# p-mc-grath/DMMFODS

Measured on AMD Instinct MI355X. Metric: training images/sec at 1280x1920 RGB+LiDAR, higher is better.
Workload: dtype f16; 1 GPU; C2 d121 early-fusion 6ch b4 1280x1920; key=c2, per_gpu_batch=4, global_batch=4, height=1280, width=1920, storage_dtype=fp16, accumulate=fp32, parallelism=dp1, weights=random-init (reference init, seed 123)

## Files before the change

### dmmfods_amd/_lib.py

```python
import ctypes as C
import os

_HERE = os.path.dirname(os.path.abspath(__file__))
LIB_PATH = os.environ.get("DMM_LIB_PATH") or os.path.join(_HERE, "libdmmfods_hip.so")

DMM_F32, DMM_F16, DMM_BF16 = 0, 1, 2
LOSS_BCE, LOSS_FOCAL = 0, 1
T_CONV, T_CONVT, T_BN_WEIGHT, T_BN_BIAS, T_BN_MEAN, T_BN_VAR, T_BN_TRACKED = range(7)
ERR_INVALID, ERR_SHAPE, ERR_HIP, ERR_STATE, ERR_NO_DEVICE = -1, -2, -3, -4, -5


class ModelDesc(C.Structure):
    _fields_ = [
        ("growth_rate", C.c_int32), ("num_blocks", C.c_int32), ("block_config", C.c_int32 * 8),
        ("num_init_features", C.c_int32), ("bn_size", C.c_int32), ("num_classes", C.c_int32),
        ("concat_before_block_num", C.c_int32), ("stream_1_in_channels", C.c_int32),
        ("stream_2_in_channels", C.c_int32), ("batch", C.c_int32), ("height", C.c_int32), ("width", C.c_int32),
        ("dtype", C.c_int32), ("loss_scale", C.c_float), ("bn_momentum", C.c_float), ("bn_eps", C.c_float),
        ("iou_threshold", C.c_float), ("use_mfma", C.c_int32),
    ]


class ConvDesc(C.Structure):
    _fields_ = [(n, C.c_int32) for n in (
        "dtype", "use_mfma", "B", "H", "W", "Cin", "Cout", "R", "S", "stride", "pad", "transposed", "mode", "bn_relu")]


class GuardState(C.Structure):
    _fields_ = [("scale", C.c_float), ("grad_scale", C.c_float), ("sumsq", C.c_double), ("grad_norm", C.c_float),
                ("found_inf", C.c_int32), ("applied_steps", C.c_int64), ("skipped_steps", C.c_int64),
                ("growth_tracker", C.c_int32), ("step_size", C.c_float), ("bc2_sqrt", C.c_float), ("clip_coef", C.c_float),
                ("reserved", C.c_int32 * 2)]


assert C.sizeof(GuardState) == 64

ADAM_MAX_CLASSES = 16


class AdamSegment(C.Structure):
    _fields_ = [("begin", C.c_int64), ("count", C.c_int64), ("cls", C.c_int32)]


class AdamClass(C.Structure):
    _fields_ = [("lr", C.c_float), ("beta1", C.c_float), ("beta2", C.c_float), ("eps", C.c_float), ("weight_decay", C.c_float),
                ("decoupled", C.c_int32), ("t0", C.c_int64)]


assert C.sizeof(AdamSegment) == 24 and C.sizeof(AdamClass) == 32


class DmmError(RuntimeError):
    pass


_lib = None


def lib():
    global _lib
    if _lib is not None:
        return _lib
    if not os.path.exists(LIB_PATH):
        raise ImportError(
            f"{LIB_PATH} is missing: build it with `python -c 'import __graft_entry__ as g; g.build()'` "
            "(or `make -C dmmfods_amd/csrc`).  dmmfods_amd has no CPU fallback.")
    import torch
    tl = os.path.join(os.path.dirname(torch.__file__), "lib", "libamdhip64.so")
    if os.path.exists(tl):
        C.CDLL(tl, mode=C.RTLD_GLOBAL)
    L = C.CDLL(LIB_PATH)
    vp, i32, i64, f32, sz = C.c_void_p, C.c_int32, C.c_int64, C.c_float, C.c_size_t
    L.dmm_last_error.restype = C.c_char_p
    L.dmm_version.restype = C.c_int
    L.dmm_last_impl.restype = C.c_int
    L.dmm_impl_name.restype = C.c_char_p
    L.dmm_impl_name.argtypes = [C.c_int]
    L.dmm_impl_mask.restype = C.c_uint
    L.dmm_impl_mask.argtypes = [C.c_int]
    L.dmm_set_option.restype = C.c_int
    L.dmm_set_option.argtypes = [C.c_char_p, C.c_int]
    L.dmm_plan_create.argtypes = [C.POINTER(ModelDesc), C.POINTER(vp)]
    L.dmm_plan_destroy.argtypes = [vp]
    L.dmm_plan_destroy.restype = C.c_int
    L.dmm_plan_num_tensors.argtypes = [vp]
    L.dmm_plan_tensor_info.argtypes = [vp, C.c_int, C.POINTER(C.c_char_p), C.POINTER(i32), C.POINTER(i32),
                                       C.POINTER(i64 * 4), C.POINTER(i64)]
    L.dmm_plan_num_params.argtypes = [vp]
    L.dmm_plan_num_params.restype = i64
    L.dmm_plan_num_buffer_elems.argtypes = [vp]
    L.dmm_plan_num_buffer_elems.restype = i64
    L.dmm_plan_workspace_bytes.argtypes = [vp]
    L.dmm_plan_workspace_bytes.restype = sz
    L.dmm_plan_forward_flops.argtypes = [vp]
    L.dmm_plan_forward_flops.restype = C.c_double
    L.dmm_plan_bind.argtypes = [vp, vp, sz, vp, vp, vp]
    L.dmm_plan_forward.argtypes = [vp, vp, vp, vp, C.c_int, vp]
    L.dmm_plan_loss_backward.argtypes = [vp, vp, vp, vp, vp]
    L.dmm_plan_backward.argtypes = [vp, vp, vp]
    L.dmm_plan_loss_metrics.argtypes = [vp, vp, vp, vp, vp]
    L.dmm_plan_set_loss.argtypes = [vp, C.c_int, vp, vp, C.c_int]
    L.dmm_loss_forward.argtypes = [C.c_int, C.c_int, vp, vp, vp, vp, vp, vp, C.c_int, C.c_int, C.c_int, C.c_int, vp]
    L.dmm_plan_num_grad_buckets.argtypes = [vp]
    L.dmm_plan_num_graph_replays.argtypes = [vp, C.c_int]
    L.dmm_plan_num_graph_replays.restype = C.c_longlong
    L.dmm_plan_grad_bucket.argtypes = [vp, C.c_int, C.POINTER(i64), C.POINTER(i64)]
    L.dmm_plan_grad_bucket_wait.argtypes = [vp, C.c_int, vp]
    L.dmm_plan_profile_begin.argtypes = [vp, C.c_int]
    L.dmm_plan_profile_filter.restype = C.c_int
    L.dmm_plan_profile_filter.argtypes = [vp, C.c_char_p]
    L.dmm_plan_profile_num_ops.argtypes = [vp, C.c_int]
    L.dmm_plan_profile_op.argtypes = [vp, C.c_int, C.c_int, C.POINTER(C.c_char_p), C.POINTER(C.c_double), C.POINTER(C.c_double)]
    L.dmm_plan_profile_collect.argtypes = [vp, C.c_int, C.POINTER(C.c_double), C.c_int, C.POINTER(C.c_int)]
    L.dmm_adam_step.argtypes = [vp, vp, vp, vp, i64, f32, f32, f32, f32, f32, i64, f32, vp]
    L.dmm_grad_guard_scratch_bytes.argtypes = [i64]
    L.dmm_grad_guard_scratch_bytes.restype = sz
    L.dmm_guard_state_init.argtypes = [vp, f32, i64, i32, vp]
    L.dmm_adam_step_guarded.argtypes = [vp, vp, vp, vp, i64, f32, f32, f32, f32, f32, f32, f32, f32, i32, vp, vp, vp]
    L.dmm_adam_step_guarded_ranges.argtypes = [vp, vp, vp, vp, C.POINTER(i64), C.POINTER(i64), C.POINTER(i64), C.c_int,
                                               f32, f32, f32, f32, f32, f32, f32, f32, i32, vp, vp, vp]
    L.dmm_plan_set_encoder_frozen.argtypes = [vp, C.c_int]
    L.dmm_adam_table_bytes.argtypes = [C.c_int, i64]
    L.dmm_adam_table_bytes.restype = sz
    L.dmm_adam_table_init.argtypes = [vp, C.POINTER(AdamSegment), C.c_int, i64, C.c_int, vp]
    L.dmm_adam_step_segmented.argtypes = [vp, vp, vp, vp, i64, vp, C.c_int, C.POINTER(AdamClass), C.c_int, i64, f32, vp]
    L.dmm_adam_step_guarded_segmented.argtypes = [vp, vp, vp, vp, i64, vp, C.c_int, C.POINTER(AdamClass), C.c_int, f32, f32, f32, i32,
                                                  vp, vp, vp]
    L.dmm_grad_sumsq.argtypes = [vp, i64, i64, C.c_int, vp, vp]
    L.dmm_plan_set_dynamic_loss_scale.argtypes = [vp, vp]
    L.dmm_plan_set_grad_accumulate.argtypes = [vp, C.c_int]
    L.dmm_conv_scratch_bytes.argtypes = [C.POINTER(ConvDesc)]
    L.dmm_conv_scratch_bytes.restype = sz
    L.dmm_conv_forward.argtypes = [C.POINTER(ConvDesc), vp, vp, vp, vp, vp, vp, vp, vp]
    L.dmm_conv_wgrad.argtypes = [C.POINTER(ConvDesc), vp, vp, vp, vp, vp, vp, vp]
    L.dmm_conv_dgrad.argtypes = [C.POINTER(ConvDesc), vp, vp, vp, vp, vp, vp, vp, vp, vp]
    L.dmm_conv_wgrad_ex.argtypes = [C.POINTER(ConvDesc), vp, vp, vp, vp, vp, vp, vp, C.c_int, vp, vp, vp]
    L.dmm_conv_dgrad_ex.argtypes = [C.POINTER(ConvDesc), vp, vp, vp, vp, vp, vp, vp, vp, vp, C.c_int, vp, vp, vp]
    L.dmm_conv1x1_backward_fused.argtypes = [C.POINTER(ConvDesc), vp, vp, vp, vp, vp, vp, vp, vp, vp, C.c_int, vp, vp, vp, vp]
    L.dmm_conv5_wgrad_stats.argtypes = [C.POINTER(ConvDesc), vp, vp, vp, vp, vp, vp, vp, vp, vp]
    L.dmm_plan_wgrad_batch_counts.argtypes = [vp, C.POINTER(C.c_longlong * 4)]
    L.dmm_conv_wgrad_grouped.argtypes = [C.POINTER(ConvDesc), C.c_int, vp, vp, vp, vp, vp, vp, vp, vp, vp, C.c_int, C.POINTER(C.c_int), vp]
    L.dmm_bw1_reduce_grouped.argtypes = [C.c_int, vp, vp, C.POINTER(C.c_int), C.POINTER(C.c_int), C.POINTER(C.c_int), C.c_int,
                                         C.POINTER(C.c_int), vp]
    _lib = L
    return L


EXPORTS = [
    "dmm_last_error", "dmm_version", "dmm_set_option", "dmm_plan_create", "dmm_plan_destroy", "dmm_plan_num_tensors",
    "dmm_plan_tensor_info", "dmm_plan_num_params", "dmm_plan_num_buffer_elems", "dmm_plan_workspace_bytes",
    "dmm_plan_forward_flops", "dmm_plan_bind", "dmm_plan_forward", "dmm_plan_loss_backward", "dmm_plan_backward",
    "dmm_plan_loss_metrics", "dmm_plan_num_graph_replays", "dmm_plan_set_loss", "dmm_loss_forward", "dmm_plan_num_grad_buckets", "dmm_plan_grad_bucket",
    "dmm_plan_grad_bucket_wait", "dmm_plan_profile_begin", "dmm_plan_profile_filter", "dmm_plan_profile_num_ops", "dmm_plan_profile_op",
    "dmm_plan_profile_collect", "dmm_adam_step", "dmm_conv_scratch_bytes", "dmm_conv_forward", "dmm_conv_wgrad",
    "dmm_conv_dgrad", "dmm_conv_wgrad_ex", "dmm_conv_dgrad_ex", "dmm_conv1x1_backward_fused", "dmm_conv5_wgrad_stats", "dmm_last_impl", "dmm_impl_name", "dmm_impl_mask",
    "dmm_grad_guard_scratch_bytes", "dmm_guard_state_init", "dmm_adam_step_guarded", "dmm_grad_sumsq", "dmm_plan_set_dynamic_loss_scale",
    "dmm_plan_set_grad_accumulate", "dmm_plan_set_encoder_frozen", "dmm_adam_step_guarded_ranges",
    "dmm_adam_table_bytes", "dmm_adam_table_init", "dmm_adam_step_segmented", "dmm_adam_step_guarded_segmented",
    "dmm_plan_wgrad_batch_counts", "dmm_conv_wgrad_grouped", "dmm_bw1_reduce_grouped",
]


def check(rc):
    if rc == 0:
        return
    msg = lib().dmm_last_error().decode(errors="replace")
    if rc == ERR_SHAPE:
        raise ValueError(msg)
    if rc == ERR_INVALID and "fusion" in msg:
        raise AttributeError(msg)
    if rc == ERR_INVALID:
        raise ValueError(msg)
    raise DmmError(f"dmm status {rc}: {msg}")


def last_impl():
    L = lib()
    return L.dmm_impl_name(L.dmm_last_impl()).decode()


def impls_since_reset(reset=True):
    L = lib()
    m = L.dmm_impl_mask(1 if reset else 0)
    return {L.dmm_impl_name(i).decode() for i in range(32) if (m >> i) & 1}


def stream_ptr():
    import torch
    return C.c_void_p(torch.cuda.current_stream().cuda_stream)
```

### dmmfods_amd/csrc/bw1.hip

```cpp
#include <algorithm>
#include <cstdio>
#include <cstring>
#include <cstdlib>
#include <type_traits>

#include "common.h"
#include "dispatch.h"
#include "gather.h"
#include "isa.h"
#include "pointwise.h"

namespace dmm {

#ifndef B1_DBG
#define B1_DBG 0
#endif
#ifndef B1_LATE_PREFETCH
#define B1_LATE_PREFETCH 0
#endif
#ifndef B1_RAW_BAR
#define B1_RAW_BAR 0
#endif
#ifndef B1_NT
#define B1_NT 0
#endif
#ifndef B1_GOLD_EARLY
#define B1_GOLD_EARLY 0
#endif
constexpr int B1_TM = 64;
constexpr int B1_NB = 128;
constexpr int B1_CT = 128;
constexpr int B1_IMG = B1_TM * 256;
constexpr int B1_W = 4 * B1_CT * 64;
constexpr int B1_STAGE = B1_TM * B1_CT * 4;
static_assert(B1_STAGE == 2 * B1_IMG, "staging aliases the operand images exactly");
constexpr int B1_LDS = 2 * B1_IMG + B1_W + 2 * B1_CT * 8 + 6 * B1_CT * 4;

__device__ __forceinline__ int b1_swz(int row, int slot) { return ((((slot >> 2) ^ (row & 3)) << 2) | ((slot & 3) ^ ((row >> 2) & 3))); }

template <typename T, int PQ, bool ACC_, bool PART>
__global__ __launch_bounds__(NTHREADS, 2) void bw1_kernel(const Bw1Args g) {
  constexpr bool ACC = ACC_ && !(B1_DBG & 32);
  constexpr bool UNC = std::is_same<T, f16>::value;
  static_assert(sizeof(T) == 2, "16-bit storage");
  typedef typename TT<T>::vec V;
  constexpr int SLOT = 8;
  constexpr int NL = B1_TM * 16 / NTHREADS;
  const ConvArgs& a = g.c;
  const Seg& sg = a.seg[0];

  extern __shared__ __attribute__((aligned(16))) unsigned char smem[];
  unsigned char* Ai = smem;
  unsigned char* Gi = smem + B1_IMG;
  unsigned char* Wi = smem + 2 * B1_IMG;
  double* red = (double*)(smem + 2 * B1_IMG + B1_W);
  float* kc = (float*)(smem + 2 * B1_IMG + B1_W + 2 * B1_CT * 8);

  const int tid = threadIdx.x, lane = tid & 63, wave = tid >> 6;
  const int r = lane & 31, h = lane >> 5;
  const int xcd = blockIdx.x & 7, q = blockIdx.x >> 3;
  const int ct = g.xcd_group ? q % g.nct : (int)(blockIdx.x % g.nct);
  const int split = g.xcd_group ? (q / g.nct) * 8 + xcd : (int)(blockIdx.x / g.nct);
  const int c0 = ct * B1_CT;
  const int t_beg = split * g.tiles_per_wg, t_end = min(g.ntiles, t_beg + g.tiles_per_wg);
  if (t_beg >= t_end) return;

  const int cs = tid & 15, p0 = tid >> 4;
  const int cx = c0 + cs * SLOT;
  const bool cvalid = cx < a.N;
  if (tid < B1_CT) {
    const int c = c0 + tid;
    const bool v = c < a.N;
    kc[tid] = v ? a.bscale[c] : 0.f; kc[B1_CT + tid] = v ? a.bshift[c] : 0.f;
    kc[2 * B1_CT + tid] = v ? a.bmean[c] : 0.f; kc[3 * B1_CT + tid] = v ? a.binvstd[c] : 0.f;
    kc[4 * B1_CT + tid] = PQ == 2 ? sg.q[tid] : 0.f; kc[5 * B1_CT + tid] = PQ == 2 ? sg.r[tid] : 0.f;
  }
  const unsigned char* xbase = (const unsigned char*)a.bx;
  const unsigned char* gbase = (const unsigned char*)sg.src;
  const unsigned char* ybase = (const unsigned char*)sg.src2;
  unsigned char* obase = (unsigned char*)a.out;
  const unsigned xcol = (unsigned)(cvalid ? cx : 0) * 2u, gcol = (unsigned)(cs * SLOT) * 2u;
  const unsigned xpitch = (unsigned)a.ldbx * 2u, gpitch = (unsigned)sg.ld * 2u, ypitch = (unsigned)sg.ld2 * 2u, opitch = (unsigned)a.ldo * 2u;
  const int lds0 = p0 * 256 + (b1_swz(p0, cs) << 4);

  {
    const T* wp = (const T*)a.wpack;
#pragma unroll
    for (int j = 0; j < B1_W / 16 / NTHREADS; ++j) {
      const int piece = tid + NTHREADS * j;
      const int chunk = piece >> 9, rowc = (piece >> 2) & 127, slot = piece & 3;
      const int c = c0 + rowc;
      V v;
#pragma unroll
      for (int e = 0; e < SLOT; ++e) v[e] = (T)0;
      if (c < a.Npad) v = *(const V*)(wp + ((size_t)chunk * a.Npad + c) * 32 + slot * SLOT);
      *(V*)(Wi + chunk * (B1_CT * 64) + rowc * 64 + ((slot ^ ((rowc >> 2) & 3)) << 4)) = v;
    }
  }
  if (tid < 2 * B1_CT) red[tid] = 0.0;
  __syncthreads();

  V rx[NL], rg[NL], ry[PQ == 2 ? NL : 1];
  unsigned okp = 0;
  auto issue = [&](int tile) {
    okp = 0;
#pragma unroll
    for (int i = 0; i < NL; ++i) {
      const int m = tile * B1_TM + p0 + 16 * i;
      if (m < a.M) okp |= 1u << i;
      const unsigned mm = (B1_DBG & 16) ? 0u : (unsigned)min(m, a.M - 1);
      if (B1_NT & 1) rx[i] = __builtin_nontemporal_load((const V*)(xbase + (size_t)(mm * xpitch + xcol)));
      else rx[i] = *(const V*)(xbase + (size_t)(mm * xpitch + xcol));
      rg[i] = *(const V*)(gbase + (size_t)(mm * gpitch + gcol));
      if constexpr (PQ == 2) ry[i] = *(const V*)(ybase + (size_t)(mm * ypitch + gcol));
    }
  };

  const int dpx = 32 * (wave & 1) + r;
  const int dgoff = dpx * 256;
  const int dcb = 64 * (wave >> 1);
  const int bsw = (r >> 2) & 3;
  const int tg = lane >> 4, ti = lane & 15, tq = ti >> 2, tp = ti & 3;
  const int arow = 8 * (tg >> 1) + tq;
  auto tr_off = [&](int px, int colbyte) { return px * 256 + ((b1_swz(px, colbyte >> 4) << 4) | (colbyte & 15)); };
  const int acolb = (32 * wave + 16 * (tg & 1) + 4 * tp) * 2;
  const int aoff1 = tr_off(arow, acolb);
  int goff1[4];
#pragma unroll
  for (int j = 0; j < 4; ++j) goff1[j] = tr_off(arow, (32 * j + 16 * (tg & 1) + 4 * tp) * 2);
  auto second = [](int off) { return (off ^ 16) + 4 * 256; };

  f32x16 accw[4];
#pragma unroll
  for (int j = 0; j < 4; ++j)
#pragma unroll
    for (int i = 0; i < 16; ++i) accw[j][i] = 0.f;

  issue(t_beg);
  for (int tile = t_beg; tile < t_end; ++tile) {
    V xraw[NL], gold[ACC ? NL : 1];
    const bool full = (tile + 1) * B1_TM <= a.M;
    const unsigned okt = okp;
    auto stage = [&](auto full_tag) {
      constexpr bool FULL = decltype(full_tag)::value;
      V z;
#pragma unroll
      for (int e = 0; e < SLOT; ++e) z[e] = (T)0;
      {
        SlotK<SLOT> kx;
        kx.k0 = load_fv<SLOT>(kc + cs * SLOT); kx.k1 = load_fv<SLOT>(kc + B1_CT + cs * SLOT); kx.k2 = 0.f; kx.k3 = 0.f;
#pragma unroll
        for (int i = 0; i < NL; ++i) {
          xraw[i] = rx[i];
          const bool v = FULL || ((okt >> i) & 1) != 0;
          const V av_ = bn_relu_slot(rx[i], kx);
          *(V*)(Ai + lds0 + 4096 * i) = v ? av_ : z;
        }
      }
      {
        SlotK<SLOT> kg;
        kg.k0 = 0.f; kg.k1 = 0.f; kg.k2 = 0.f; kg.k3 = 0.f;
        if (PQ == 2) { kg.k0 = load_fv<SLOT>(kc + 4 * B1_CT + cs * SLOT); kg.k1 = load_fv<SLOT>(kc + 5 * B1_CT + cs * SLOT); }
#pragma unroll
        for (int i = 0; i < NL; ++i) {
          const bool v = FULL || ((okt >> i) & 1) != 0;
          V gv = rg[i];
          if constexpr (PQ == 2) gv = eff_grad_slot(rg[i], ry[i], kg);
          *(V*)(Gi + lds0 + 4096 * i) = v ? gv : z;
        }
      }
    };
    if (UNC && full) stage(std::true_type()); else stage(std::false_type());
    __syncthreads();
#if !B1_LATE_PREFETCH
    if (tile + 1 < t_end) issue(tile + 1);
#endif
#if B1_GOLD_EARLY
    if constexpr (ACC) {
#pragma unroll
      for (int i = 0; i < NL; ++i) {
        const unsigned mm = (unsigned)min(tile * B1_TM + p0 + 16 * i, a.M - 1);
        gold[i] = *(const V*)(obase + (size_t)(mm * opitch + xcol));
      }
    }
#endif

    f32x16 accd[2];
#pragma unroll
    for (int t = 0; t < 2; ++t)
#pragma unroll
      for (int i = 0; i < 16; ++i) accd[t][i] = 0.f;
    if (!(B1_DBG & 4))
#pragma unroll
    for (int ch = 0; ch < 4; ++ch)
#pragma unroll
      for (int s = 0; s < 2; ++s) {
        const int slot = ch * 4 + 2 * s + h;
        const V av = *(const V*)(Gi + dgoff + (b1_swz(dpx, slot) << 4));
#pragma unroll
        for (int t = 0; t < 2; ++t) {
          const V bv = *(const V*)(Wi + ch * (B1_CT * 64) + (dcb + 32 * t + r) * 64 + (((2 * s + h) ^ bsw) << 4));
          accd[t] = mma16(av, bv, accd[t]);
        }
      }
    if (!(B1_DBG & 2))
#pragma unroll
    for (int ms = 0; ms < B1_TM / 16; ++ms) {
      const V af = frag16<T>(lds_tr16(Ai + aoff1 + ms * 4096), lds_tr16(Ai + second(aoff1) + ms * 4096));
#pragma unroll
      for (int j = 0; j < 4; ++j) {
        const V gf = frag16<T>(lds_tr16(Gi + goff1[j] + ms * 4096), lds_tr16(Gi + second(goff1[j]) + ms * 4096));
        accw[j] = mma16(gf, af, accw[j]);
      }
    }
#if !B1_GOLD_EARLY
    if constexpr (ACC) {
#pragma unroll
      for (int i = 0; i < NL; ++i) {
        const unsigned mm = (unsigned)min(tile * B1_TM + p0 + 16 * i, a.M - 1);
        if (B1_NT & 1) gold[i] = __builtin_nontemporal_load((const V*)(obase + (size_t)(mm * opitch + xcol)));
        else gold[i] = *(const V*)(obase + (size_t)(mm * opitch + xcol));
      }
    }
#endif
#if B1_LATE_PREFETCH
    if (tile + 1 < t_end) issue(tile + 1);
#endif
#if B1_RAW_BAR
    lds_barrier();
#else
    __syncthreads();
#endif
    if (B1_DBG & 8) {
      float sa = 0.f;
#pragma unroll
      for (int t = 0; t < 2; ++t)
#pragma unroll
        for (int i = 0; i < 16; ++i) sa += accd[t][i];
      if (sa == 1.2345e33f) obase[0] = 1;
    } else {
    float* Cs = (float*)smem;
#pragma unroll
    for (int t = 0; t < 2; ++t)
#pragma unroll
      for (int i = 0; i < 16; ++i) {
        const int row = 32 * (wave & 1) + (i & 3) + 8 * (i >> 2) + 4 * h;
        Cs[row * B1_CT + ((dcb + 32 * t + r) ^ (h << 5))] = accd[t][i];
      }
#if B1_RAW_BAR
    lds_barrier();
#else
    __syncthreads();
#endif
    float s1[SLOT], s2[SLOT];
#pragma unroll
    for (int e = 0; e < SLOT; ++e) { s1[e] = 0.f; s2[e] = 0.f; }
    auto finish = [&](auto full_tag) {
      constexpr bool FULL = decltype(full_tag)::value;
      float sc[SLOT], sh[SLOT], mu[UNC ? 1 : SLOT], is[UNC ? 1 : SLOT];
      load_f32s<SLOT>(kc + cs * SLOT, sc); load_f32s<SLOT>(kc + B1_CT + cs * SLOT, sh);
      if constexpr (!UNC) { load_f32s<SLOT>(kc + 2 * B1_CT + cs * SLOT, mu); load_f32s<SLOT>(kc + 3 * B1_CT + cs * SLOT, is); }
#pragma unroll
      for (int i = 0; i < NL; ++i) {
        if (!FULL && !((okt >> i) & 1)) continue;
        const int p = p0 + 16 * i;
        float av[SLOT];
#pragma unroll
        for (int e = 0; e < SLOT; e += 4) {
          const f32x4 t4 = *(const f32x4*)(Cs + p * B1_CT + ((cs * SLOT + e) ^ (((p >> 2) & 1) << 5)));
          av[e] = t4[0]; av[e + 1] = t4[1]; av[e + 2] = t4[2]; av[e + 3] = t4[3];
        }
        const unsigned m = (unsigned)(tile * B1_TM + p);
        if constexpr (UNC) {
          const V ov = bnbwd_slot<ACC>(av, xraw[i], gold[ACC ? i : 0], sc, sh, s1, s2);
          if (B1_NT & 2) __builtin_nontemporal_store(ov, (V*)(obase + (size_t)(m * opitch + xcol)));
          else if (!(B1_DBG & 64) || av[0] == 1.2345e33f) *(V*)(obase + (size_t)(m * opitch + xcol)) = ov;
        } else {
          float xf[SLOT], gf[SLOT];
          vec_to_f32<T>(xraw[i], xf);
          if constexpr (ACC) vec_to_f32<T>(gold[i], gf);
#pragma unroll
          for (int e = 0; e < SLOT; ++e) {
            const float dz = (fmaf(xf[e], sc[e], sh[e]) > 0.f) ? av[e] : 0.f;
            s1[e] += dz;
            s2[e] = fmaf(dz, (xf[e] - mu[e]) * is[e], s2[e]);
            gf[e] = (ACC ? gf[e] : 0.f) + sc[e] * dz;
          }
          if (!(B1_DBG & 64) || gf[0] == 1.2345e33f) *(V*)(obase + (size_t)(m * opitch + xcol)) = f32_to_vec<T>(gf);
        }
      }
    };
    if (cvalid) { if (UNC && full) finish(std::true_type()); else finish(std::false_type()); }
    fold_to_lds<16, SLOT, B1_CT>(s1, s2, red, cs, cvalid, lane);
    }
#if B1_RAW_BAR
    lds_barrier();
#else
    __syncthreads();
#endif
  }

  if (tid < B1_CT && c0 + tid < a.N) {
    const size_t rep = (size_t)(blockIdx.x & (STAT_REPS - 1)) * a.stat_stride;
    const double S1 = red[fold_slot<16, SLOT>(0, tid)];
    double S2 = red[fold_slot<16, SLOT>(1, tid)];
    if constexpr (UNC) S2 = (S2 - (double)kc[2 * B1_CT + tid] * S1) * (double)kc[3 * B1_CT + tid];
    atomic_add_f64(a.red1 + rep + c0 + tid, S1);
    atomic_add_f64(a.red2 + rep + c0 + tid, S2);
  }
  const int c = c0 + 32 * wave + r;
  if constexpr (PART) {
    float* slot = g.part + ((size_t)split * g.nct + ct) * B1_SLOT_FLOATS + (size_t)wave * (B1_NB * 32);
#pragma unroll
    for (int j = 0; j < 4; ++j)
#pragma unroll
      for (int i = 0; i < 16; ++i) {
        const int n = 32 * j + (i & 3) + 8 * (i >> 2) + 4 * h;
        slot[n * 32 + r] = accw[j][i];
      }
  } else if (!(B1_DBG & 1) && c < g.wC) {
    const size_t chunk = (size_t)(c0 / 32 + wave);
#pragma unroll
    for (int j = 0; j < 4; ++j)
#pragma unroll
      for (int i = 0; i < 16; ++i) {
        const int n = 32 * j + (i & 3) + 8 * (i >> 2) + 4 * h;
        atomic_add_f32(g.dpack + (chunk * g.dNpad + n) * 32 + r, accw[j][i]);
      }
  }
  if (B1_DBG & 1) {
    float s = 0.f;
#pragma unroll
    for (int j = 0; j < 4; ++j)
#pragma unroll
      for (int i = 0; i < 16; ++i) s += accw[j][i];
    if (s == 1.2345e33f) g.dpack[0] = s;
  }
}

template <typename T, int PQ, bool ACC, bool PART>
static hipError_t launch_bw1_t(const Bw1Args& g, int nwg, hipStream_t st) {
  return launch_lds<bw1_kernel<T, PQ, ACC, PART>>(B1_LDS, nwg, NTHREADS, B1_LDS, st, g);
}

bool bw1_eligible(const WgradArgs& w, const ConvArgs& d, int dtype, unsigned deny) {
  if (((deny >> IMPL_BW1) & 1u) || dtype == DT_F32 || w.nseg != 1 || d.nseg != 1 || d.pool2) return false;
  const Seg& wx = w.seg[0];
  const Seg& wg = w.dy;
  const Seg& dg = d.seg[0];
  if (wx.mode != G_PLAIN || wx.istride != 1 || wx.ntaps != 1 || wx.taps[0] != 0 || wx.scale == nullptr || wx.C % 32) return false;
  if (wg.mode != G_PLAIN || wg.istride != 1 || wg.ntaps != 1 || wg.taps[0] != 0 || wg.scale != nullptr || wg.C != B1_NB) return false;
  if (dg.mode != G_PLAIN || dg.istride != 1 || dg.ntaps != 1 || dg.taps[0] != 0 || dg.scale != nullptr || dg.C != B1_NB || dg.Cpad != B1_NB) return false;
  if (dg.src != wg.src || dg.ld != wg.ld || dg.q != wg.q || dg.src2 != wg.src2) return false;
  if (w.N != B1_NB || w.Npad != B1_NB || w.M != d.M || d.N != wx.C || d.Npad % 32) return false;
  if (d.bx != wx.src || d.ldbx != wx.ld || d.bscale != wx.scale || d.bshift != wx.shift) return false;
  if (d.out == nullptr || d.ostride != 1 || d.Hout != d.Ho || d.Wout != d.Wo || wx.Hs != d.Ho || wx.Ws != d.Wo) return false;
  const double span = 2.0 * (double)d.M;
  if (span * d.ldbx >= 4294967296.0 || span * d.ldo >= 4294967296.0 || span * dg.ld >= 4294967296.0 || span * dg.ld2 >= 4294967296.0) return false;
  return true;
}

Bw1Geom bw1_geometry(const ConvArgs& a) {
  Bw1Geom q;
  q.nct = (a.N + B1_CT - 1) / B1_CT;
  q.ntiles = (a.M + B1_TM - 1) / B1_TM;
  constexpr int cus = DESIGN_CUS;
  static const int per_cu = lab_int("DMM_BW1_PER_CU", 2);
  int nsplit = std::max(1, (per_cu * cus + q.nct - 1) / q.nct);
  nsplit = std::min(nsplit, std::max(1, q.ntiles / 4));
  q.tiles_per_wg = (q.ntiles + nsplit - 1) / nsplit;
  q.nsplit = (q.ntiles + q.tiles_per_wg - 1) / q.tiles_per_wg;
  q.xcd_group = (q.nct > 1 && q.nsplit >= 32 && q.tiles_per_wg >= 8) ? 1 : 0;
  q.nwg = q.xcd_group ? ((q.nsplit + 7) / 8) * 8 * q.nct : q.nsplit * q.nct;
  return q;
}

static bool g_bw1_part = !lab_flag("DMM_NO_BW1_PART");

static bool bw1_uses_part(const Bw1Args& g, const Bw1Geom& q) {
  return g_bw1_part && g.part != nullptr && q.nsplit * q.nct <= g.part_slots && q.nsplit > 1;
}

hipError_t launch_bw1(const Bw1Args& g0, int dtype, hipStream_t st) {
  Bw1Args g = g0;
  const ConvArgs& a = g.c;
  if (a.M <= 0) return hipSuccess;
  const Bw1Geom q = bw1_geometry(a);
  note_impl(IMPL_BW1);
  g.nct = q.nct; g.ntiles = q.ntiles; g.tiles_per_wg = q.tiles_per_wg; g.xcd_group = q.xcd_group; g.nsplit = q.nsplit;
  const int nwg = q.nwg;
  const int pq = a.seg[0].q ? 2 : 0;
  const bool acc = a.accumulate != 0;
  const bool part = bw1_uses_part(g, q);
#define B1_GO(T) \
  (part ? (pq ? (acc ? launch_bw1_t<T, 2, true, true>(g, nwg, st) : launch_bw1_t<T, 2, false, true>(g, nwg, st))     \
              : (acc ? launch_bw1_t<T, 0, true, true>(g, nwg, st) : launch_bw1_t<T, 0, false, true>(g, nwg, st)))    \
        : (pq ? (acc ? launch_bw1_t<T, 2, true, false>(g, nwg, st) : launch_bw1_t<T, 2, false, false>(g, nwg, st))   \
              : (acc ? launch_bw1_t<T, 0, true, false>(g, nwg, st) : launch_bw1_t<T, 0, false, false>(g, nwg, st))))
  if (dtype == DT_F16) return B1_GO(f16);
  return B1_GO(bf16);
#undef B1_GO
}

__device__ __forceinline__ void bw1_reduce_slots(const float* __restrict__ part, float* __restrict__ dpack, int nct, int nsplit, int nfloats) {
  const int e = (blockIdx.x * 256 + threadIdx.x) * 4;
  if (e >= nct * B1_SLOT_FLOATS) return;
  f32x4 s = {0.f, 0.f, 0.f, 0.f};
  const float* p = part + e;
  const size_t pitch = (size_t)nct * B1_SLOT_FLOATS;
  int k = 0;
  for (; k + 16 <= nsplit; k += 16) {
    f32x4 v[16];
#pragma unroll
    for (int u = 0; u < 16; ++u) v[u] = __builtin_nontemporal_load((const f32x4*)(p + (size_t)(k + u) * pitch));
#pragma unroll
    for (int u = 0; u < 16; u += 4) s += (v[u] + v[u + 1]) + (v[u + 2] + v[u + 3]);
  }
  for (; k + 4 <= nsplit; k += 4) {
    const f32x4 v0 = *(const f32x4*)(p + (size_t)k * pitch), v1 = *(const f32x4*)(p + (size_t)(k + 1) * pitch);
    const f32x4 v2 = *(const f32x4*)(p + (size_t)(k + 2) * pitch), v3 = *(const f32x4*)(p + (size_t)(k + 3) * pitch);
    s += (v0 + v1) + (v2 + v3);
  }
  for (; k < nsplit; ++k) s += *(const f32x4*)(p + (size_t)k * pitch);
  if (e < nfloats) *(f32x4*)(dpack + e) = s;
}
__global__ __launch_bounds__(256) void bw1_reduce_kernel(const float* __restrict__ part, float* __restrict__ dpack, int nct, int nsplit, int nfloats) {
  bw1_reduce_slots(part, dpack, nct, nsplit, nfloats);
}
struct Bw1RedGroupArgs { Bw1RedMember m[B1_RED_GROUP_MAX]; };
static_assert(sizeof(Bw1RedMember) % 8 == 0, "members are read with aligned scalar loads");
__global__ __launch_bounds__(256) void bw1_reduce_group_kernel(const Bw1RedGroupArgs g) {
  const Bw1RedMember& m = g.m[blockIdx.y];
  bw1_reduce_slots(m.part, m.dpack, m.nct, m.nsplit, m.nfloats);
}

static bool bw1_reduce_member(const Bw1Args& g, Bw1RedMember& m) {
  const ConvArgs& a = g.c;
  if (a.M <= 0) return false;
  const Bw1Geom q = bw1_geometry(a);
  if (!bw1_uses_part(g, q)) return false;
  m.part = g.part; m.dpack = g.dpack; m.nct = q.nct; m.nsplit = q.nsplit;
  m.nfloats = ((g.wC + 31) / 32) * g.dNpad * 32;
  return true;
}

hipError_t launch_bw1_reduce_member(const Bw1RedMember& m, hipStream_t st) {
  const int nthreads = m.nct * B1_SLOT_FLOATS / 4;
  hipLaunchKernelGGL(bw1_reduce_kernel, dim3((nthreads + 255) / 256), dim3(256), 0, st, m.part, m.dpack, m.nct, m.nsplit, m.nfloats);
  return hipGetLastError();
}

hipError_t launch_bw1_reduce(const Bw1Args& g, hipStream_t st) {
  Bw1RedMember m;
  if (!bw1_reduce_member(g, m)) return hipSuccess;
  return launch_bw1_reduce_member(m, st);
}

bool bw1_reduce_group_add(Bw1RedGroup& G, const Bw1Args& g) {
  Bw1RedMember m;
  if (!bw1_reduce_member(g, m)) return true;
  if (G.n >= B1_RED_GROUP_MAX) return false;
  G.m[G.n++] = m;
  return true;
}

hipError_t bw1_reduce_group_launch(Bw1RedGroup& G, hipStream_t st) {
  if (G.n <= 0) return hipSuccess;
  Bw1RedGroupArgs a;
  memset(&a, 0, sizeof(a));
  int nct = 0;
  for (int i = 0; i < G.n; ++i) { a.m[i] = G.m[i]; nct = std::max(nct, G.m[i].nct); }
  const int n = G.n;
  G.n = 0;
  hipLaunchKernelGGL(bw1_reduce_group_kernel, dim3((nct * (B1_SLOT_FLOATS / 4) + 255) / 256, n), dim3(256), 0, st, a);
  return hipGetLastError();
}

}
```

### dmmfods_amd/csrc/capi.cpp

```cpp
#include <algorithm>
#include <atomic>
#include <cmath>
#include <cstdio>
#include <cstdlib>
#include <cstring>
#include <stdexcept>
#include <chrono>
#include <mutex>
#include <string>
#include <utility>
#include <vector>
#include <unistd.h>

#include "dispatch.h"
#include "plan.h"

using namespace dmm;

void plan_build_tables(dmm_plan* p);
void plan_bind(dmm_plan* p, void* ws);
void plan_size(dmm_plan* p);

static thread_local std::string g_err;
static int fail(int code, const std::string& msg) {
  g_err = msg;
  return code;
}
#define HIPCHK(expr)                                                                                   \
  do {                                                                                                 \
    hipError_t e__ = (expr);                                                                           \
    if (e__ != hipSuccess) return fail(DMM_ERR_HIP, std::string(#expr) + ": " + hipGetErrorString(e__)); \
  } while (0)

static bool g_overlap_wgrad = getenv("DMM_NO_OVERLAP") == nullptr;
static int g_graph = getenv("DMM_GRAPH") ? std::max(1, atoi(getenv("DMM_GRAPH"))) : 0;
static unsigned long long g_option_epoch = 1;
static int g_batch_wgrad = 1;
static int g_bucket_mb = getenv("DMM_GRAD_BUCKET_MB") ? atoi(getenv("DMM_GRAD_BUCKET_MB")) : 25;
static std::atomic<unsigned> g_family_off{lab_family_off()};
static unsigned plan_deny(const dmm_plan* p) { return (p->sw.no_hf ? 1u << IMPL_HF : 0u) | g_family_off; }

namespace {
struct DevicePool {
  std::mutex mu;
  hipStream_t side = nullptr, pack = nullptr, capture = nullptr;
  std::vector<hipEvent_t> free_plain, free_timing;
  long events_made = 0;
};
constexpr int MAX_DEVICES = 64;
DevicePool* g_pools[MAX_DEVICES] = {};
std::mutex g_pools_mu;

DevicePool* pool_of(int device) {
  if (device < 0 || device >= MAX_DEVICES) return nullptr;
  std::lock_guard<std::mutex> l(g_pools_mu);
  if (g_pools[device] == nullptr) g_pools[device] = new DevicePool();
  return g_pools[device];
}
hipError_t pool_streams(DevicePool* dp, bool want_capture) {
  std::lock_guard<std::mutex> l(dp->mu);
  if (dp->side == nullptr) {
    int lo = 0, hi = 0;
    hipError_t e = hipDeviceGetStreamPriorityRange(&lo, &hi);
    if (e != hipSuccess) return e;
    hipStream_t s = nullptr, k = nullptr;
    if ((e = hipStreamCreateWithPriority(&s, hipStreamNonBlocking, lo)) != hipSuccess) return e;
    if ((e = hipStreamCreateWithPriority(&k, hipStreamNonBlocking, lo)) != hipSuccess) return e;
    dp->side = s; dp->pack = k;
  }
  if (want_capture && dp->capture == nullptr) {
    hipStream_t c = nullptr;
    const hipError_t e = hipStreamCreateWithFlags(&c, hipStreamNonBlocking);
    if (e != hipSuccess) return e;
    dp->capture = c;
  }
  return hipSuccess;
}
hipEvent_t pool_event(DevicePool* dp, bool timing) {
  std::lock_guard<std::mutex> l(dp->mu);
  auto& fl = timing ? dp->free_timing : dp->free_plain;
  if (!fl.empty()) { hipEvent_t e = fl.back(); fl.pop_back(); return e; }
  hipEvent_t e = nullptr;
  const hipError_t rc = timing ? hipEventCreate(&e) : hipEventCreateWithFlags(&e, hipEventDisableTiming);
  if (rc != hipSuccess) return nullptr;
  ++dp->events_made;
  return e;
}
void pool_return(DevicePool* dp, std::vector<void*>& evs, bool timing) {
  std::lock_guard<std::mutex> l(dp->mu);
  auto& fl = timing ? dp->free_timing : dp->free_plain;
  for (void* e : evs) if (e) fl.push_back((hipEvent_t)e);
  evs.clear();
}
void trace_destroy(const char* what) {
  static const bool on = getenv("DMM_TRACE_DESTROY") != nullptr;
  if (!on) return;
  char buf[160];
  const int n = snprintf(buf, sizeof(buf), "[dmm] destroy: %s\n", what);
  if (n > 0) { ssize_t w = write(2, buf, (size_t)std::min<int>(n, (int)sizeof(buf) - 1)); (void)w; }
}
}

extern "C" {

const char* dmm_last_error(void) { return g_err.c_str(); }
int dmm_version(void) { return 101; }

static const char* const kImplNames[IMPL_COUNT] = {"auto", "generic", "thin", "conv3", "cvp", "halo", "wg3", "wg5", "wgp", "pig", "bw1", "hf", "cf", "wgpw", "cvw"};
static const struct { const char* option; int family; } kFamilyOptions[] = {
    {"thin_logits", IMPL_THIN}, {"conv3", IMPL_CONV3}, {"wg3", IMPL_WG3}, {"wgp", IMPL_WGP},
    {"wg5", IMPL_WG5},          {"cvp", IMPL_CVP},     {"bw1", IMPL_BW1}, {"pig", IMPL_PIG},
};

int dmm_set_option(const char* name, int value) {
  if (!name) return fail(DMM_ERR_INVALID, "null argument");
  ++g_option_epoch;
  if (std::string(name) == "overlap_wgrad") { g_overlap_wgrad = value != 0; return DMM_OK; }
  if (std::string(name) == "graph") { g_graph = value; return DMM_OK; }
  if (std::string(name) == "batch_wgrad") {
    if (value < 0 || value > 2) return fail(DMM_ERR_INVALID, "batch_wgrad must be 0, 1 or 2");
    g_batch_wgrad = value;
    return DMM_OK;
  }
  for (const auto& o : kFamilyOptions)
    if (std::string(name) == o.option) {
      if (value != 0) g_family_off &= ~(1u << o.family);
      else g_family_off |= 1u << o.family;
      return DMM_OK;
    }
  if (std::string(name) == "grad_bucket_mb") {
    if (value < 0) return fail(DMM_ERR_INVALID, "grad_bucket_mb must be >= 0");
    g_bucket_mb = value;
    return DMM_OK;
  }
  return fail(DMM_ERR_INVALID, std::string("unknown option ") + name);
}

int dmm_plan_create(const dmm_model_desc* desc, dmm_plan** out) {
  if (!desc || !out) return fail(DMM_ERR_INVALID, "null argument");
  if (desc->num_blocks < 2 || desc->num_blocks > 8) return fail(DMM_ERR_INVALID, "num_blocks must be in [2, 8]");
  if (desc->dtype != DMM_F32 && desc->dtype != DMM_F16 && desc->dtype != DMM_BF16)
    return fail(DMM_ERR_INVALID, "dtype must be DMM_F32, DMM_F16 or DMM_BF16");
  if (desc->dtype == DMM_BF16 && !desc->use_mfma) return fail(DMM_ERR_INVALID, "DMM_BF16 has no scalar check kernels: use_mfma must be 1");
  if (desc->batch < 1) return fail(DMM_ERR_INVALID, "batch must be >= 1");
  if (!(desc->loss_scale > 0)) return fail(DMM_ERR_INVALID, "loss_scale must be > 0");
  dmm_plan* p = new dmm_plan();
  p->desc = *desc;
  p->sw = PlanSwitches::from_environment();
  p->bucket_bytes = (size_t)g_bucket_mb << 20;
  p->deny = plan_deny(p);
  try {
    plan_build_tables(p);
  } catch (const std::domain_error& e) {
    delete p;
    return fail(DMM_ERR_SHAPE, e.what());
  } catch (const std::exception& e) {
    delete p;
    return fail(DMM_ERR_INVALID, e.what());
  }
  *out = p;
  return DMM_OK;
}

int dmm_plan_destroy(dmm_plan* plan) {
  if (!plan) return DMM_OK;
  trace_destroy("begin");
  std::string first_err;
  auto note = [&](hipError_t e, const char* what) {
    if (e != hipSuccess && first_err.empty()) first_err = std::string(what) + ": " + hipGetErrorString(e);
  };
  DevicePool* dp = plan->device >= 0 ? pool_of(plan->device) : nullptr;
  if (dp != nullptr) {
    int cur = -1;
    const bool switched = hipGetDevice(&cur) == hipSuccess && cur != plan->device && hipSetDevice(plan->device) == hipSuccess;
    if (plan->used_side) {
      trace_destroy("synchronise the side stream");
      note(hipStreamSynchronize(dp->side), "hipStreamSynchronize(side stream)");
      trace_destroy("synchronise the pack stream");
      note(hipStreamSynchronize(dp->pack), "hipStreamSynchronize(pack stream)");
    }
    if (plan->used_capture && dp->capture) {
      trace_destroy("synchronise the capture stream");
      note(hipStreamSynchronize(dp->capture), "hipStreamSynchronize(capture stream)");
    }
    trace_destroy("graphs");
    for (auto& gc : plan->graphs) {
      for (auto& e : gc.entries) note(hipGraphExecDestroy((hipGraphExec_t)e.exec), "hipGraphExecDestroy");
      gc.entries.clear();
    }
    trace_destroy("events back to the pool");
    pool_return(dp, plan->fork_events, false);
    pool_return(dp, plan->join_events, false);
    pool_return(dp, plan->bucket_events, false);
    for (auto& which : plan->prof_events)
      for (auto& pass : which) pool_return(dp, pass, true);
    if (switched) (void)hipSetDevice(cur);
  }
  trace_destroy("delete");
  delete plan;
  trace_destroy("done");
  return first_err.empty() ? DMM_OK : fail(DMM_ERR_HIP, "dmm_plan_destroy: " + first_err);
}

int dmm_plan_num_tensors(const dmm_plan* plan) { return plan ? (int)plan->tensors.size() : 0; }

int dmm_plan_tensor_info(const dmm_plan* plan, int index, const char** name, int32_t* kind, int32_t* ndim, int64_t shape[4],
                         int64_t* arena_offset) {
  if (!plan || index < 0 || index >= (int)plan->tensors.size()) return fail(DMM_ERR_INVALID, "tensor index out of range");
  const TensorInfo& t = plan->tensors[index];
  if (name) *name = t.name.c_str();
  if (kind) *kind = t.kind;
  if (ndim) *ndim = t.ndim;
  if (shape) for (int i = 0; i < 4; ++i) shape[i] = t.shape[i];
  if (arena_offset) *arena_offset = t.off;
  return DMM_OK;
}

int64_t dmm_plan_num_params(const dmm_plan* plan) { return plan ? plan->nparams : 0; }
int64_t dmm_plan_num_buffer_elems(const dmm_plan* plan) { return plan ? plan->nbuf : 0; }
size_t dmm_plan_workspace_bytes(const dmm_plan* plan) { return plan ? plan->zero_bytes + plan->zero_bwd_bytes + plan->main_bytes : 0; }
double dmm_plan_forward_flops(const dmm_plan* plan) { return plan ? plan->fwd_flops : 0; }

int dmm_plan_bind(dmm_plan* plan, void* workspace, size_t workspace_bytes, float* params, float* grads, float* buffers) {
  if (!plan || !workspace || !params || !grads || !buffers) return fail(DMM_ERR_INVALID, "null argument");
  if (workspace_bytes < dmm_plan_workspace_bytes(plan)) return fail(DMM_ERR_INVALID, "workspace too small");
  if ((uintptr_t)workspace % 256) return fail(DMM_ERR_INVALID, "workspace must be 256-byte aligned");
  int ndev = 0;
  if (hipGetDeviceCount(&ndev) != hipSuccess || ndev == 0) return fail(DMM_ERR_NO_DEVICE, "no HIP device");
  int dev = 0;
  HIPCHK(hipGetDevice(&dev));
  if (plan->device >= 0 && plan->device != dev) return fail(DMM_ERR_STATE, "the plan is bound to another device");
  if (dev >= MAX_DEVICES) return fail(DMM_ERR_INVALID, "device index out of range");
  plan->device = dev;
  plan->params = params;
  plan->grads = grads;
  plan->buffers = buffers;
  plan->graphs[0].epoch = plan->graphs[1].epoch = 0;
  plan->bound = false;
  plan->deny = plan_deny(plan);
  try {
    plan_bind(plan, workspace);
  } catch (const dmm::plan_sizing_error& e) {
    return fail(DMM_ERR_STATE, e.what());
  } catch (const std::exception& e) {
    return fail(DMM_ERR_INVALID, e.what());
  }
  HIPCHK(hipDeviceSynchronize());
  plan->bound = true;
  return DMM_OK;
}

static std::string family_check(const Op& o, unsigned ran) {
  if ((o.kind == OP_IGEMM ? o.c.M : o.w.M) <= 0) return std::string();
  const bool recorded_ran = (ran >> o.impl) & 1u;
  const bool generic_ran = (ran >> IMPL_GENERIC) & 1u;
  const bool wgp_remainder = o.kind == OP_WGRAD && o.impl == IMPL_WGP && o.w.nseg == 2 && o.w.nphase == 0;
  if (recorded_ran && (o.impl == IMPL_GENERIC || !generic_ran || wgp_remainder)) return std::string();
  std::string names;
  for (int f = 1; f < IMPL_COUNT; ++f)
    if ((ran >> f) & 1u) names += (names.empty() ? "" : "+") + std::string(dmm_impl_name(f));
  return std::string("launch '") + o.label + "': the plan recorded family " + dmm_impl_name(o.impl) + ", " + (names.empty() ? "none" : names) + " ran";
}

static int run_ops(dmm_plan* p, std::vector<Op>& ops, hipStream_t st, int prof_which = -1, size_t begin = 0, size_t end = 0, bool capturing = false) {
  if (end == 0 || end > ops.size()) end = ops.size();
  const size_t ev_offset = 0;
  const int dt = p->desc.dtype;
  const bool mfma = p->desc.use_mfma != 0;
  std::vector<void*>* evs = nullptr;
  if (prof_which >= 0 && p->prof_max_passes > 0 && p->prof_pass[prof_which] < p->prof_max_passes) {
    auto& sets = p->prof_events[prof_which];
    const int pass = p->prof_pass[prof_which]++;
    if ((int)sets.size() <= pass) sets.resize(pass + 1);
    evs = &sets[pass];
    const size_t need = 2 * (ops.size() + ev_offset);
    DevicePool* pdp = pool_of(p->device);
    while (evs->size() < need) {
      hipEvent_t e = pdp ? pool_event(pdp, true) : nullptr;
      if (e == nullptr) return fail(DMM_ERR_HIP, "hipEventCreate failed");
      evs->push_back((void*)e);
    }
  }
  const bool accumulate = p->grad_accumulate;
  const std::string& filt = p->prof_filter;
  auto selected = [&](const Op& o) { return evs != nullptr && (filt.empty() || strncmp(o.label, filt.c_str(), filt.size()) == 0); };
  const bool overlap = g_overlap_wgrad && !capturing && (evs == nullptr || !filt.empty());
  constexpr int nside = 1;
  size_t nfork = 0;
  bool forked = false;
  DevicePool* dp = pool_of(p->device);
  hipStream_t side_st = nullptr, pack_st = nullptr;
  if (overlap) {
    if (dp == nullptr || pool_streams(dp, false) != hipSuccess) return fail(DMM_ERR_HIP, "side stream");
    side_st = dp->side; pack_st = dp->pack;
    while ((int)p->join_events.size() < nside + 1) {
      hipEvent_t je = pool_event(dp, false);
      if (je == nullptr) return fail(DMM_ERR_HIP, "hipEventCreate failed");
      p->join_events.push_back((void*)je);
    }
    p->used_side = true;
  }
  bool pack_pending = false;
  auto join_pack = [&]() {
    if (pack_pending) {
      hipStreamWaitEvent(st, (hipEvent_t)p->join_events[nside], 0);
      pack_pending = false;
    }
  };
  auto join_side = [&]() {
    if (forked) {
      for (int k = 0; k < nside; ++k) {
        hipEventRecord((hipEvent_t)p->join_events[k], side_st);
        hipStreamWaitEvent(st, (hipEvent_t)p->join_events[k], 0);
      }
      forked = false;
    }
  };
  auto join = [&]() { join_side(); join_pack(); };
  const bool batch = g_batch_wgrad != 0;
  static const long long w3_batch_tiles = lab_int("DMM_WG3_BATCH_TILES", 0);
  Wg3Group w3g;
  Bw1RedGroup rdg;
  std::vector<size_t> w3_members, rd_members;
  const bool batch_main = g_batch_wgrad == 1;
  hipStream_t batch_st = (overlap && !batch_main) ? side_st : st;
  auto flush_members = [&](std::vector<size_t>& members, auto&& launch) -> hipError_t {
    if (members.empty()) return hipSuccess;
    for (size_t k = 0; k + 1 < members.size(); ++k)
      if (selected(ops[members[k]])) {
        hipEventRecord((hipEvent_t)(*evs)[2 * (ev_offset + members[k])], batch_st);
        hipEventRecord((hipEvent_t)(*evs)[2 * (ev_offset + members[k]) + 1], batch_st);
      }
    const size_t last = members.back();
    const bool sel_last = selected(ops[last]);
    members.clear();
    if (sel_last) hipEventRecord((hipEvent_t)(*evs)[2 * (ev_offset + last)], batch_st);
    const hipError_t fe = launch();
    if (sel_last) hipEventRecord((hipEvent_t)(*evs)[2 * (ev_offset + last) + 1], batch_st);
    return fe;
  };
  auto flush_w3 = [&]() { return flush_members(w3_members, [&] { ++p->batch_counts[0]; return wg3_group_launch(w3g, batch_st); }); };
  auto flush_rd = [&]() { return flush_members(rd_members, [&] { ++p->batch_counts[2]; return bw1_reduce_group_launch(rdg, batch_st); }); };
  auto flush_all = [&]() { const hipError_t e1 = flush_w3(), e2 = flush_rd(); return e1 != hipSuccess ? e1 : e2; };
  auto flush_failed = [&](hipError_t fe) { join(); return fail(DMM_ERR_HIP, std::string("grouped weight-gradient launch: ") + hipGetErrorString(fe)); };
  static const bool host_prof = lab_flag("DMM_HOST_PROF");
  static double hp_launch[32] = {0}, hp_fork[32] = {0};
  static long hp_n[32] = {0}, hp_lists = 0;
  auto now = [] { return std::chrono::duration<double, std::micro>(std::chrono::steady_clock::now().time_since_epoch()).count(); };
  for (size_t i = begin; i < end; ++i) {
    Op& o = ops[i];
    hipError_t e = hipSuccess;
    const double hp_t0 = host_prof ? now() : 0.0;
    double hp_t1 = hp_t0;
    const bool forks = !o.chain && o.leaf != 2 && o.leaf != 3 && (o.kind == OP_WGRAD || o.leaf);
    bool as_w3 = false, as_rd = false;
    if (batch && forks && o.signal < 0) {
      if (o.kind == OP_WGRAD && o.impl == IMPL_WG3 && mfma) {
        as_w3 = wg3_group_add(w3g, o.w, dt);
        if (!as_w3 && w3g.n > 0) {
          if ((e = flush_w3()) != hipSuccess) return flush_failed(e);
          as_w3 = wg3_group_add(w3g, o.w, dt);
        }
      } else if (o.kind == OP_BW1RED) {
        as_rd = bw1_reduce_group_add(rdg, o.b1);
        if (!as_rd) {
          if ((e = flush_rd()) != hipSuccess) return flush_failed(e);
          as_rd = bw1_reduce_group_add(rdg, o.b1);
        }
      }
    }
    const bool rd_added = as_rd && rdg.n > (int)rd_members.size();
    if (!as_w3 && !as_rd && (forks || o.leaf == 3 || o.signal >= 0 || (o.kind == OP_JOIN && o.epi != 1)))
      if ((e = flush_all()) != hipSuccess) return flush_failed(e);
    hipStream_t lst = st;
    if (overlap && o.leaf == 3 && forked) {
      lst = side_st;
    } else if (batch_main && forks && ((o.kind == OP_WGRAD && o.impl == IMPL_WG3) || o.kind == OP_BW1RED)) {
    } else if (overlap && !o.chain && (o.kind == OP_WGRAD || o.leaf)) {
      if (nfork >= p->fork_events.size()) {
        hipEvent_t fe = pool_event(dp, false);
        if (fe == nullptr) { join(); return fail(DMM_ERR_HIP, "hipEventCreate failed"); }
        p->fork_events.push_back((void*)fe);
      }
      lst = o.leaf == 2 ? pack_st : side_st;
      hipEvent_t fe = (hipEvent_t)p->fork_events[nfork++];
      hipEventRecord(fe, st);
      hipStreamWaitEvent(lst, fe, 0);
      if (o.leaf == 2) pack_pending = true; else forked = true;
      if (host_prof) hp_t1 = now();
    }
    const bool sel = selected(o) && !as_w3 && !rd_added;
// ... 198 lines not shown
  if (metrics_out) HIPCHK(hipMemcpyAsync(metrics_out, plan->metrics, plan->metrics_bytes, hipMemcpyDeviceToDevice, (hipStream_t)stream));
  return DMM_OK;
}

int dmm_plan_backward(dmm_plan* plan, const float* dlogits, void* stream) {
  if (!plan || !plan->bound) return fail(DMM_ERR_STATE, "plan not bound");
  if (!dlogits) return fail(DMM_ERR_INVALID, "null argument");
  hipStream_t st = (hipStream_t)stream;
  const BceArgs& b = plan->bwd[plan->bce_op].bce;
  ConvertArgs cv;
  memset(&cv, 0, sizeof(cv));
  cv.src1 = dlogits; cv.C1 = b.NC; cv.dst = b.dlogits; cv.B = b.B; cv.H = b.H; cv.W = b.W;
  cv.scale = plan->desc.loss_scale;
  cv.dyn_scale = plan->dyn_scale;
  int rc = run_ops(plan, plan->bwd, st, -1, 0, (size_t)plan->bce_op);
  if (rc) return rc;
  HIPCHK(launch_convert_input(cv, plan->desc.dtype, st));
  return run_ops(plan, plan->bwd, st, -1, (size_t)plan->bce_op + 1, 0);
}

int dmm_plan_wgrad_batch_counts(const dmm_plan* plan, long long counts[4]) {
  if (!plan || !counts) return fail(DMM_ERR_INVALID, "null argument");
  for (int i = 0; i < 4; ++i) counts[i] = plan->batch_counts[i];
  return DMM_OK;
}

long long dmm_plan_num_graph_replays(const dmm_plan* plan, int which) {
  return (plan && which >= 0 && which <= 1) ? plan->graph_replays[which] : 0;
}

int dmm_plan_num_grad_buckets(const dmm_plan* plan) { return plan ? (int)plan->buckets.size() : 0; }

int dmm_plan_grad_bucket(const dmm_plan* plan, int index, int64_t* offset, int64_t* count) {
  if (!plan || index < 0 || index >= (int)plan->buckets.size()) return fail(DMM_ERR_INVALID, "bucket index out of range");
  if (offset) *offset = plan->buckets[index].off;
  if (count) *count = plan->buckets[index].n;
  return DMM_OK;
}

int dmm_plan_grad_bucket_wait(dmm_plan* plan, int index, void* stream) {
  if (!plan || index < 0 || index >= (int)plan->buckets.size()) return fail(DMM_ERR_INVALID, "bucket index out of range");
  const GradBucket& b = plan->buckets[index];
  plan->dp_used = true;
  for (int ev : {b.ev_main, b.ev_side}) {
    if (ev < 0) continue;
    if (ev >= (int)plan->bucket_events.size()) return fail(DMM_ERR_STATE, "no backward pass has been enqueued on this plan yet");
    HIPCHK(hipStreamWaitEvent((hipStream_t)stream, (hipEvent_t)plan->bucket_events[ev], 0));
  }
  return DMM_OK;
}

int dmm_plan_profile_begin(dmm_plan* plan, int max_passes) {
  if (!plan) return fail(DMM_ERR_INVALID, "null plan");
  plan->prof_max_passes = max_passes;
  plan->prof_pass[0] = plan->prof_pass[1] = 0;
  return DMM_OK;
}

int dmm_plan_profile_filter(dmm_plan* plan, const char* label_prefix) {
  if (!plan) return fail(DMM_ERR_INVALID, "null plan");
  plan->prof_filter = label_prefix ? label_prefix : "";
  return DMM_OK;
}

int dmm_plan_profile_num_ops(const dmm_plan* plan, int which) {
  if (!plan || which < 0 || which > 1) return 0;
  return (int)(which == 0 ? plan->fwd_train.size() : plan->bwd.size());
}

int dmm_plan_profile_op(const dmm_plan* plan, int which, int index, const char** label, double* flops, double* bytes) {
  if (!plan || which < 0 || which > 1) return fail(DMM_ERR_INVALID, "bad argument");
  const std::vector<Op>& ops = which == 0 ? plan->fwd_train : plan->bwd;
  if (index < 0 || index >= (int)ops.size()) return fail(DMM_ERR_INVALID, "op index out of range");
  if (label) *label = ops[index].label;
  if (flops) *flops = ops[index].flops;
  if (bytes) *bytes = ops[index].bytes;
  return DMM_OK;
}

int dmm_plan_profile_collect(dmm_plan* plan, int which, double* ms_sum, int n, int* passes) {
  if (!plan || which < 0 || which > 1 || !ms_sum) return fail(DMM_ERR_INVALID, "bad argument");
  const int nops = dmm_plan_profile_num_ops(plan, which);
  if (n < nops) return fail(DMM_ERR_INVALID, "buffer too small");
  for (int i = 0; i < nops; ++i) ms_sum[i] = 0;
  int np = 0;
  for (auto& evs : plan->prof_events[which]) {
    if ((int)evs.size() < 2 * nops || np >= plan->prof_pass[which]) continue;
    const std::vector<Op>& ops = which == 0 ? plan->fwd_train : plan->bwd;
    const std::string& filt = plan->prof_filter;
    for (int i = 0; i < nops; ++i) {
      if (!filt.empty() && strncmp(ops[i].label, filt.c_str(), filt.size()) != 0) continue;
      float ms = 0;
      if (hipEventElapsedTime(&ms, (hipEvent_t)evs[2 * i], (hipEvent_t)evs[2 * i + 1]) != hipSuccess) return fail(DMM_ERR_HIP, "hipEventElapsedTime failed");
      ms_sum[i] += ms;
    }
    ++np;
  }
  if (passes) *passes = np;
  return DMM_OK;
}

int dmm_plan_loss_metrics(dmm_plan* plan, const float* logits, const float* target, double* metrics_out, void* stream) {
  if (!plan || !plan->bound) return fail(DMM_ERR_STATE, "plan not bound");
  if (!logits || !target || !metrics_out) return fail(DMM_ERR_INVALID, "null argument");
  hipStream_t st = (hipStream_t)stream;
  HIPCHK(hipMemsetAsync(plan->metrics, 0, plan->metrics_bytes, st));
  Op o = plan->bce_only;
  o.bce.logits = logits;
  o.bce.target = target;
  set_loss_fields(plan, o.bce);
  HIPCHK(launch_bce_metrics(o.bce, plan->desc.dtype, st));
  HIPCHK(hipMemcpyAsync(metrics_out, plan->metrics, plan->metrics_bytes, hipMemcpyDeviceToDevice, st));
  return DMM_OK;
}

int dmm_adam_step(float* params, const float* grads, float* exp_avg, float* exp_avg_sq, int64_t n, float lr, float beta1, float beta2,
                  float eps, float weight_decay, int64_t step, float grad_scale, void* stream) {
  if (!params || !grads || !exp_avg || !exp_avg_sq || n < 0 || step < 1) return fail(DMM_ERR_INVALID, "bad Adam argument");
  AdamArgs a;
  a.p = params; a.g = grads; a.m = exp_avg; a.v = exp_avg_sq; a.n = (size_t)n;
  a.beta1 = beta1; a.beta2 = beta2; a.eps = eps; a.weight_decay = weight_decay;
  const double bc1 = 1.0 - std::pow((double)beta1, (double)step), bc2 = 1.0 - std::pow((double)beta2, (double)step);
  a.step_size = (float)(lr / bc1);
  a.bc2_sqrt = (float)std::sqrt(bc2);
  a.grad_scale = grad_scale;
  HIPCHK(launch_adam(a, (hipStream_t)stream));
  return DMM_OK;
}

int dmm_plan_set_dynamic_loss_scale(dmm_plan* plan, const float* scale_dev) {
  if (!plan) return fail(DMM_ERR_INVALID, "null plan");
  if (((uintptr_t)scale_dev & 3) != 0) return fail(DMM_ERR_INVALID, "dynamic loss scale pointer must be 4-byte aligned");
  plan->dyn_scale = scale_dev;
  if (plan->bound && plan->bce_op >= 0) plan->bwd[plan->bce_op].bce.dyn_scale = scale_dev;
  return DMM_OK;
}

int dmm_plan_set_grad_accumulate(dmm_plan* plan, int accumulate) {
  if (!plan) return fail(DMM_ERR_INVALID, "null plan");
  const bool on = accumulate != 0;
  if (on == plan->grad_accumulate) return DMM_OK;
  plan->grad_accumulate = on;
  plan->graphs[1].epoch = 0;
  return DMM_OK;
}

int dmm_plan_set_encoder_frozen(dmm_plan* plan, int frozen) {
  if (!plan) return fail(DMM_ERR_INVALID, "null plan");
  if (plan->bound) return fail(DMM_ERR_STATE, "dmm_plan_set_encoder_frozen: the plan is bound (set the mode between dmm_plan_create and dmm_plan_bind)");
  const bool on = frozen != 0;
  if (on == plan->encoder_frozen) return DMM_OK;
  plan->encoder_frozen = on;
  plan->deny = plan_deny(plan);
  try {
    plan_size(plan);
  } catch (const std::exception& e) {
    plan->encoder_frozen = !on;
    try { plan_size(plan); } catch (...) {}
    return fail(DMM_ERR_INVALID, e.what());
  }
  return DMM_OK;
}

size_t dmm_grad_guard_scratch_bytes(int64_t n) {
  (void)n;
  return (size_t)GUARD_PARTIALS * sizeof(double);
}

int dmm_guard_state_init(dmm_guard_state* dev, float init_scale, int64_t applied_steps, int32_t growth_tracker, void* stream) {
  if (!dev) return fail(DMM_ERR_INVALID, "null guard state");
  if (((uintptr_t)dev & 7) != 0) return fail(DMM_ERR_INVALID, "guard state must be 8-byte aligned");
  if (!(init_scale > 0.f) || !std::isfinite(init_scale)) return fail(DMM_ERR_INVALID, "init_scale must be a finite number > 0");
  if (applied_steps < 0 || growth_tracker < 0) return fail(DMM_ERR_INVALID, "applied_steps and growth_tracker must be >= 0");
  HIPCHK(launch_guard_init(dev, init_scale, applied_steps, growth_tracker, (hipStream_t)stream));
  return DMM_OK;
}

int dmm_grad_sumsq(const float* grads, int64_t offset, int64_t count, int accumulate, void* scratch, void* stream) {
  if (!grads || !scratch) return fail(DMM_ERR_INVALID, "null argument");
  if (offset < 0 || count < 0) return fail(DMM_ERR_INVALID, "offset and count must be >= 0");
  if ((((uintptr_t)grads) & 3) != 0 || (((uintptr_t)scratch) & 7) != 0) return fail(DMM_ERR_INVALID, "misaligned gradient or scratch pointer");
  GradSumsqArgs r;
  r.g = grads + offset; r.n = (size_t)count; r.partials = (double*)scratch; r.accumulate = accumulate ? 1 : 0;
  HIPCHK(launch_grad_sumsq(r, (hipStream_t)stream));
  return DMM_OK;
}

int dmm_adam_step_guarded(float* params, const float* grads, float* exp_avg, float* exp_avg_sq, int64_t n, float lr, float beta1,
                          float beta2, float eps, float weight_decay, float max_norm, float growth_factor, float backoff_factor,
                          int32_t growth_interval, dmm_guard_state* state, void* scratch, void* stream) {
  if (!params || !grads || !exp_avg || !exp_avg_sq || !state || !scratch) return fail(DMM_ERR_INVALID, "null argument of the guarded Adam step");
  if (n < 0) return fail(DMM_ERR_INVALID, "n must be >= 0");
  if ((((uintptr_t)grads) & 3) != 0 || (((uintptr_t)state) & 7) != 0 || (((uintptr_t)scratch) & 7) != 0)
    return fail(DMM_ERR_INVALID, "misaligned gradient, state or scratch pointer");
  if (!(growth_factor >= 1.f) || !std::isfinite(growth_factor)) return fail(DMM_ERR_INVALID, "growth_factor must be a finite number >= 1");
  if (!(backoff_factor > 0.f) || !(backoff_factor <= 1.f)) return fail(DMM_ERR_INVALID, "backoff_factor must lie in (0, 1]");
  if (growth_interval < 0) return fail(DMM_ERR_INVALID, "growth_interval must be >= 0");
  if (std::isnan(max_norm)) return fail(DMM_ERR_INVALID, "max_norm is NaN");
  if (!(beta1 >= 0.f && beta1 < 1.f) || !(beta2 >= 0.f && beta2 < 1.f)) return fail(DMM_ERR_INVALID, "betas must lie in [0, 1)");
  hipStream_t st = (hipStream_t)stream;
  GradSumsqArgs r;
  r.g = grads; r.n = (size_t)n; r.partials = (double*)scratch; r.accumulate = 0;
  HIPCHK(launch_grad_sumsq(r, st));
  GuardFinalizeArgs f;
  f.partials = (const double*)scratch; f.state = state; f.lr = lr; f.beta1 = beta1; f.beta2 = beta2; f.max_norm = max_norm;
  f.growth_factor = growth_factor; f.backoff_factor = backoff_factor; f.growth_interval = growth_interval;
  HIPCHK(launch_guard_finalize(f, st));
  AdamArgs a;
  a.p = params; a.g = grads; a.m = exp_avg; a.v = exp_avg_sq; a.n = (size_t)n;
  a.beta1 = beta1; a.beta2 = beta2; a.eps = eps; a.weight_decay = weight_decay;
  a.step_size = 0.f; a.bc2_sqrt = 1.f; a.grad_scale = 0.f;
  HIPCHK(launch_adam_guarded(a, state, st));
  return DMM_OK;
}

int dmm_adam_step_guarded_ranges(float* params, const float* grads, float* exp_avg, float* exp_avg_sq, const int64_t* offsets,
                                 const int64_t* counts, const int64_t* t0, int nranges, float lr, float beta1, float beta2, float eps,
                                 float weight_decay, float max_norm, float growth_factor, float backoff_factor, int32_t growth_interval,
                                 dmm_guard_state* state, void* scratch, void* stream) {
  if (!params || !grads || !exp_avg || !exp_avg_sq || !offsets || !counts || !t0 || !state || !scratch)
    return fail(DMM_ERR_INVALID, "null argument of the guarded Adam step over ranges");
  if (nranges < 1) return fail(DMM_ERR_INVALID, "nranges must be >= 1");
  if ((((uintptr_t)grads) & 3) != 0 || (((uintptr_t)state) & 7) != 0 || (((uintptr_t)scratch) & 7) != 0)
    return fail(DMM_ERR_INVALID, "misaligned gradient, state or scratch pointer");
  for (int i = 0; i < nranges; ++i) {
    if (offsets[i] < 0 || counts[i] < 0) return fail(DMM_ERR_INVALID, "range " + std::to_string(i) + ": offset and count must be >= 0");
    if (t0[i] < 0) return fail(DMM_ERR_INVALID, "range " + std::to_string(i) + ": t0 must be >= 0");
    if (offsets[i] > INT64_MAX - counts[i]) return fail(DMM_ERR_INVALID, "range " + std::to_string(i) + ": offset + count overflows");
    for (int k = 0; k < i; ++k)
      if (offsets[i] < offsets[k] + counts[k] && offsets[k] < offsets[i] + counts[i])
        return fail(DMM_ERR_INVALID, "ranges " + std::to_string(k) + " and " + std::to_string(i) + " overlap");
  }
  if (!(growth_factor >= 1.f) || !std::isfinite(growth_factor)) return fail(DMM_ERR_INVALID, "growth_factor must be a finite number >= 1");
  if (!(backoff_factor > 0.f) || !(backoff_factor <= 1.f)) return fail(DMM_ERR_INVALID, "backoff_factor must lie in (0, 1]");
  if (growth_interval < 0) return fail(DMM_ERR_INVALID, "growth_interval must be >= 0");
  if (std::isnan(max_norm)) return fail(DMM_ERR_INVALID, "max_norm is NaN");
  if (!(beta1 >= 0.f && beta1 < 1.f) || !(beta2 >= 0.f && beta2 < 1.f)) return fail(DMM_ERR_INVALID, "betas must lie in [0, 1)");
  hipStream_t st = (hipStream_t)stream;
  for (int i = 0; i < nranges; ++i) {
    GradSumsqArgs r;
    r.g = grads + offsets[i]; r.n = (size_t)counts[i]; r.partials = (double*)scratch; r.accumulate = i > 0 ? 1 : 0;
    HIPCHK(launch_grad_sumsq(r, st));
  }
  GuardFinalizeArgs f;
  f.partials = (const double*)scratch; f.state = state; f.lr = lr; f.beta1 = beta1; f.beta2 = beta2; f.max_norm = max_norm;
  f.growth_factor = growth_factor; f.backoff_factor = backoff_factor; f.growth_interval = growth_interval;
  HIPCHK(launch_guard_finalize(f, st));
  for (int i = 0; i < nranges; ++i) {
    AdamArgs a;
    a.p = params + offsets[i]; a.g = grads + offsets[i]; a.m = exp_avg + offsets[i]; a.v = exp_avg_sq + offsets[i]; a.n = (size_t)counts[i];
    a.beta1 = beta1; a.beta2 = beta2; a.eps = eps; a.weight_decay = weight_decay;
    a.step_size = 0.f; a.bc2_sqrt = 1.f; a.grad_scale = 0.f;
    if (t0[i] == 0) HIPCHK(launch_adam_guarded(a, state, st));
    else HIPCHK(launch_adam_guarded_from(a, state, lr, t0[i], st));
  }
  return DMM_OK;
}

namespace {
hipError_t upload(void* dst, const void* src, size_t bytes, hipStream_t st);
struct AdamTableHost {
  int nsegs = 0, nclasses = 0;
  int64_t n = 0;
  std::vector<std::pair<int64_t, int64_t>> runs;
};
std::mutex g_adam_tables_mu;
std::vector<std::pair<const void*, AdamTableHost>> g_adam_tables;

size_t adam_table_chunks(int64_t n) { return (size_t)((n + ADAM_SEG_CHUNK - 1) / ADAM_SEG_CHUNK); }

bool bad_scalar(float x) { return std::isnan(x) || x < 0.f; }

int adam_seg_check(const char* who, const float* params, const float* grads, const float* exp_avg, const float* exp_avg_sq, int64_t n,
                   const void* table_dev, int nsegs, const dmm_adam_class* classes, int nclasses, AdamTableHost* host) {
  const std::string w(who);
  if (!params || !grads || !exp_avg || !exp_avg_sq || !table_dev || !classes) return fail(DMM_ERR_INVALID, w + ": null argument");
  if ((((uintptr_t)params | (uintptr_t)grads | (uintptr_t)exp_avg | (uintptr_t)exp_avg_sq) & 3) != 0 || ((uintptr_t)table_dev & 7) != 0)
    return fail(DMM_ERR_INVALID, w + ": misaligned arena (4 bytes) or table (8 bytes) pointer");
  if (n < 1) return fail(DMM_ERR_INVALID, w + ": n must be >= 1");
  if (nsegs < 1) return fail(DMM_ERR_INVALID, w + ": nsegs must be >= 1");
  if (nclasses < 1 || nclasses > ADAM_MAX_CLASSES)
    return fail(DMM_ERR_INVALID, w + ": nclasses must lie in [1, " + std::to_string(ADAM_MAX_CLASSES) + "]");
  for (int c = 0; c < nclasses; ++c) {
    const dmm_adam_class& k = classes[c];
    const std::string cw = w + ": class " + std::to_string(c) + ": ";
    if (!(k.beta1 >= 0.f && k.beta1 < 1.f) || !(k.beta2 >= 0.f && k.beta2 < 1.f)) return fail(DMM_ERR_INVALID, cw + "betas must lie in [0, 1)");
    if (bad_scalar(k.lr)) return fail(DMM_ERR_INVALID, cw + "lr must be >= 0 and not NaN");
    if (bad_scalar(k.eps)) return fail(DMM_ERR_INVALID, cw + "eps must be >= 0 and not NaN");
    if (bad_scalar(k.weight_decay)) return fail(DMM_ERR_INVALID, cw + "weight_decay must be >= 0 and not NaN");
    if (k.t0 < 0) return fail(DMM_ERR_INVALID, cw + "t0 must be >= 0");
  }
  std::lock_guard<std::mutex> l(g_adam_tables_mu);
  for (const auto& e : g_adam_tables)
    if (e.first == table_dev) {
      if (e.second.nsegs != nsegs || e.second.n != n)
        return fail(DMM_ERR_INVALID, w + ": table_dev was initialised for nsegs = " + std::to_string(e.second.nsegs) + ", n = " + std::to_string(e.second.n));
      if (e.second.nclasses != nclasses)
        return fail(DMM_ERR_INVALID, w + ": table_dev was initialised for nclasses = " + std::to_string(e.second.nclasses));
      *host = e.second;
      return DMM_OK;
    }
  return fail(DMM_ERR_INVALID, w + ": table_dev was not initialised by dmm_adam_table_init");
}

void adam_seg_args(AdamSegArgs& a, float* params, const float* grads, float* exp_avg, float* exp_avg_sq, int64_t n, const void* table_dev,
                   int nsegs, const dmm_adam_class* classes, int nclasses) {
// ... 359 lines not shown
int dmm_conv5_wgrad_stats(const dmm_conv_desc* d, const void* x, const void* dy, const float* w, const float* scale, const float* shift,
                          float* dw, double* red, void* scratch, void* stream) {
  OneConv g;
  if (!d || !geometry(d, g)) return fail(DMM_ERR_INVALID, "unsupported conv descriptor");
  if (d->transposed || d->mode != 0 || d->stride != 1 || d->R != 5 || d->S != 5 || d->pad != 2 || !d->bn_relu || d->Cin != 64 || d->Cout > 4 ||
      d->dtype == DMM_F32 || !d->use_mfma)
    return fail(DMM_ERR_INVALID, "serves the 5x5 convolution of 64 channels onto <= 4 behind BN+ReLU in 16-bit storage");
  hipStream_t st = (hipStream_t)stream;
  const size_t wn = (size_t)d->Cin * d->Cout * 25;
  const std::vector<Tap> taps = taps_conv_dgrad(5, 5, 2);
  Scratch S{(uint8_t*)scratch};
  PackDesc* dd = (PackDesc*)S.take(sizeof(PackDesc));
  int* dp = (int*)S.take(sizeof(int));
  PackDesc pd = dgrad_pack_desc(d, g, taps, dw, 64);
  const size_t elems = (size_t)pd.seg[0].nchunks * pd.Npad * g.BK;
  pd.dpack = (float*)S.take(elems * sizeof(float));
  pd.gw = dw;
  float* sbuf = (float*)S.take((size_t)W5_SBUF64_FLOATS * sizeof(float));
  if (S.off > dmm_conv_scratch_bytes(d)) return fail(DMM_ERR_INVALID, "scratch too small");
  HIPCHK(hipMemsetAsync(scratch, 0, S.off, st));
  HIPCHK(hipMemsetAsync(red, 0, 2 * (size_t)d->Cin * sizeof(double), st));
  int zero = 0;
  HIPCHK(upload(dd, &pd, sizeof(pd), st));
  HIPCHK(upload(dp, &zero, sizeof(int), st));
  HIPCHK(hipStreamSynchronize(st));
  WgradArgs a;
  memset(&a, 0, sizeof(a));
  a.nseg = 1;
  Seg& sq = a.seg[0];
  sq.src = dy; sq.ld = d->Cout; sq.Hs = g.Hout; sq.Ws = g.Wout; sq.C = rup(d->Cout, 8); sq.Cpad = sq.C; sq.mode = G_PLAIN; sq.istride = 1;
  fill_seg_taps(sq, taps, g.BK);
  a.B = d->B; a.Ho = g.Ho; a.Wo = g.Wo; a.M = d->B * g.Ho * g.Wo;
  fill_one_seg(a.dy, d, g, x, scale, shift, taps_conv(1, 1, 0));
  a.dy.istride = 1;
  a.N = g.Cst; a.Npad = pd.Npad;
  a.dpack = (float*)pd.dpack;
  a.sbuf = sbuf;
  a.t_mean = shift + d->Cin; a.t_invstd = shift + 2 * d->Cin;
  HIPCHK(launch_wgrad(a, d->dtype, true, st, IMPL_AUTO, g_family_off));
  if (g_last_impl != IMPL_WG5) return fail(DMM_ERR_STATE, "the factor form is wg5.hip's");
  Fin64Args f;
  memset(&f, 0, sizeof(f));
  f.sbuf = sbuf; f.dpack = a.dpack; f.Npad = a.Npad;
  f.w = w; f.Kin = d->Cin; f.nreal = d->Cout; f.dtype = d->dtype;
  for (int t = 0; t < 25; ++t) f.tapw[t] = (unsigned char)(pd.seg[0].tapw[t] & 0xff);
  f.scale = scale; f.shift = shift; f.mean = shift + d->Cin; f.invstd = shift + 2 * d->Cin;
  f.red1 = red; f.red2 = red + d->Cin;
  HIPCHK(launch_wg5_fin64(f, st));
  HIPCHK(hipMemsetAsync(dw, 0, wn * sizeof(float), st));
  HIPCHK(launch_unpack(dd, dp, 1, pd.seg[0].nchunks * pd.Npad, d->dtype, 1.0f, st));
  return DMM_OK;
}

int dmm_conv_wgrad(const dmm_conv_desc* d, const void* x, const void* dy, const float* scale, const float* shift, float* dw, void* scratch,
                   void* stream) {
  return dmm_conv_wgrad_ex(d, x, dy, scale, shift, nullptr, nullptr, nullptr, 0, dw, scratch, stream);
}

static int build_dgrad(const dmm_conv_desc* d, const OneConv& g, const void* x, const void* dy, const float* w, const float* scale,
                       const float* shift, const void* yfwd, const float* q, const float* r, void* gx, int accumulate, double* red,
                       Scratch& S, int npad, ConvArgs& a, hipStream_t st) {
  std::vector<Tap> taps;
  int istride = 1, rH = d->H, rW = d->W, pool2 = 0, ostride = 1;
  if (d->transposed) { taps = taps_convT_dgrad(); istride = 2; }
  else if (d->mode == 2) { taps = taps_conv(1, 1, 0); rH = d->H / 2; rW = d->W / 2; pool2 = 1; ostride = 2; }
  else if (d->mode == 1) { taps = taps_up2_merged_dgrad(); istride = 2; }
  else taps = taps_conv_dgrad(d->R, d->S, d->pad);
  PackDesc* dd = (PackDesc*)S.take(sizeof(PackDesc));
  int* dp = (int*)S.take(sizeof(int));
  float* zeros = (float*)S.take((size_t)rup(d->Cout, 8) * sizeof(float) + 64);
  PackDesc pd = dgrad_pack_desc(d, g, taps, w, npad);
  pd.dst = S.take((size_t)pd.seg[0].nchunks * pd.Npad * g.BK * g.esz);
  if (S.off > dmm_conv_scratch_bytes(d)) return fail(DMM_ERR_INVALID, "scratch too small");
  int zero = 0;
  HIPCHK(hipMemsetAsync(zeros, 0, (size_t)rup(d->Cout, 8) * sizeof(float) + 64, st));
  HIPCHK(upload(dd, &pd, sizeof(pd), st));
  HIPCHK(upload(dp, &zero, sizeof(int), st));
  HIPCHK(hipStreamSynchronize(st));
  HIPCHK(launch_pack(dd, dp, 1, pd.seg[0].nchunks * pd.Npad, d->dtype, st));
  HIPCHK(hipMemsetAsync(red, 0, 2 * d->Cin * sizeof(double), st));
  memset(&a, 0, sizeof(a));
  a.nseg = 1;
  Seg& s = a.seg[0];
  const int kc = rup(d->Cout, 8);
  s.src = dy; s.ld = d->Cout; s.Hs = g.Hout; s.Ws = g.Wout; s.C = kc; s.Cpad = kc; s.mode = G_PLAIN; s.istride = istride;
  set_eff_grad(s, yfwd, d->Cout, q, r, zeros);
  fill_seg_taps(s, taps, g.BK);
  a.B = d->B; a.Ho = rH; a.Wo = rW; a.M = d->B * rH * rW;
  a.wpack = pd.dst; a.N = d->Cin; a.Npad = pd.Npad;
  a.out = gx; a.ldo = d->Cin; a.Hout = d->H; a.Wout = d->W; a.ostride = ostride;
  a.bx = x; a.ldbx = d->Cin; a.bscale = scale; a.bshift = shift;
  a.bmean = shift + d->Cin; a.binvstd = shift + 2 * d->Cin;
  a.red1 = red; a.red2 = red + d->Cin;
  a.accumulate = accumulate ? 1 : 0; a.pool2 = pool2;
  return DMM_OK;
}

int dmm_conv_dgrad_ex(const dmm_conv_desc* d, const void* x, const void* dy, const float* w, const float* scale, const float* shift,
                      const void* yfwd, const float* q, const float* r, void* gx, int accumulate, double* red, void* scratch,
                      void* stream) {
  OneConv g;
  if (!d || !geometry(d, g) || !d->bn_relu) return fail(DMM_ERR_INVALID, "unsupported conv descriptor (dgrad needs bn_relu)");
  if (d->mode == 0 && !d->transposed && d->stride != 1) return fail(DMM_ERR_INVALID, "strided conv dgrad is not on the hot path");
  if ((q != nullptr) != (r != nullptr) || (q != nullptr && yfwd == nullptr)) return fail(DMM_ERR_INVALID, "q, r and yfwd come together");
  hipStream_t st = (hipStream_t)stream;
  Scratch S{(uint8_t*)scratch};
  ConvArgs a;
  const int cs = g.Cst;
  const int npad = rup(cs, cs >= 384 || cs % 128 == 0 ? 128 : (cs >= 64 ? 64 : 32));
  const int rc = build_dgrad(d, g, x, dy, w, scale, shift, yfwd, q, r, gx, accumulate, red, S, npad, a, st);
  if (rc) return rc;
  HIPCHK(launch_igemm(a, d->dtype, EPI_BNBWD, d->use_mfma != 0, st, IMPL_AUTO, g_family_off));
  return DMM_OK;
}

int dmm_conv_dgrad(const dmm_conv_desc* d, const void* x, const void* dy, const float* w, const float* scale, const float* shift, void* gx,
                   double* red, void* scratch, void* stream) {
  return dmm_conv_dgrad_ex(d, x, dy, w, scale, shift, nullptr, nullptr, nullptr, gx, 0, red, scratch, stream);
}

int dmm_conv1x1_backward_fused(const dmm_conv_desc* d, const void* x, const void* dy, const float* w, const float* scale,
                               const float* shift, const void* yfwd, const float* q, const float* r, void* gx, int accumulate,
                               float* dw, double* red, void* scratch, void* stream) {
  OneConv g;
  if (!d || !geometry(d, g) || !d->bn_relu || d->R != 1 || d->S != 1 || d->stride != 1 || d->transposed || d->mode != 0)
    return fail(DMM_ERR_INVALID, "the fused backward serves 1x1 unit-stride convolutions behind BN+ReLU");
  if ((q != nullptr) != (r != nullptr) || (q != nullptr && yfwd == nullptr)) return fail(DMM_ERR_INVALID, "q, r and yfwd come together");
  hipStream_t st = (hipStream_t)stream;
  std::vector<PackDesc> packs;
  std::vector<int> prefix;
  PackDesc* dd; int* dp; int total_rows;
  const size_t used = layout_fwd(d, g, (uint8_t*)scratch, dw, dw, packs, &dd, &dp, prefix, total_rows);
  HIPCHK(hipMemsetAsync(scratch, 0, used, st));
  HIPCHK(upload(dd, packs.data(), packs.size() * sizeof(PackDesc), st));
  HIPCHK(upload(dp, prefix.data(), prefix.size() * sizeof(int), st));
  Scratch S{(uint8_t*)scratch, used};
  Bw1Args b;
  memset(&b, 0, sizeof(b));
  const int cs = g.Cst;
  const int npad = rup(cs, cs >= 384 || cs % 128 == 0 ? 128 : (cs >= 64 ? 64 : 32));
  const int rc = build_dgrad(d, g, x, dy, w, scale, shift, yfwd, q, r, gx, accumulate, red, S, npad, b.c, st);
  if (rc) return rc;
  WgradArgs wa;
  memset(&wa, 0, sizeof(wa));
  wa.nseg = 1;
  fill_one_seg(wa.seg[0], d, g, x, scale, shift, g.phase_taps[0]);
  wa.B = d->B; wa.Ho = g.Ho; wa.Wo = g.Wo; wa.M = d->B * g.Ho * g.Wo;
  wa.dy = b.c.seg[0];
  wa.N = d->Cout; wa.Npad = packs[0].Npad;
  wa.dpack = (float*)packs[0].dpack;
  if (!bw1_eligible(wa, b.c, d->dtype, g_family_off)) return fail(DMM_ERR_INVALID, "not a pair bw1.hip fuses (16-bit storage, 128 output channels, Cin % 32 == 0)");
  b.dpack = wa.dpack; b.dNpad = wa.Npad; b.wC = wa.seg[0].C;
  {
    const Bw1Geom q = bw1_geometry(b.c);
    b.part_slots = q.nsplit * q.nct;
    void* part = nullptr;
    HIPCHK(hipMallocAsync(&part, (size_t)b.part_slots * B1_SLOT_FLOATS * sizeof(float), st));
    b.part = (float*)part;
    const hipError_t e1 = launch_bw1(b, d->dtype, st);
    const hipError_t e2 = e1 == hipSuccess ? launch_bw1_reduce(b, st) : e1;
    hipFreeAsync(part, st);
    HIPCHK(e2);
  }
  const size_t wn = (size_t)d->Cin * d->Cout;
  HIPCHK(hipMemsetAsync(dw, 0, wn * sizeof(float), st));
  HIPCHK(launch_unpack(dd, dp, (int)packs.size(), total_rows, d->dtype, 1.0f, st));
  return DMM_OK;
}

int dmm_conv_wgrad_grouped(const dmm_conv_desc* descs, int n, const void* const* x, const void* const* dy, const float* const* scale,
                           const float* const* shift, const void* const* yfwd, const float* const* q, const float* const* r,
                           float* const* dw, void* const* scratch, int grouped, int* launches, void* stream) {
  if (!descs || n < 1 || !x || !dy || !scale || !shift || !dw || !scratch) return fail(DMM_ERR_INVALID, "null argument");
  hipStream_t st = (hipStream_t)stream;
  struct One { WgradArgs a; PackDesc* dd; int* dp; int rows; };
  std::vector<One> v((size_t)n);
  for (int i = 0; i < n; ++i) {
    const dmm_conv_desc* d = &descs[i];
    OneConv g;
    if (!geometry(d, g)) return fail(DMM_ERR_INVALID, "unsupported conv descriptor");
    const void* yf = yfwd ? yfwd[i] : nullptr;
    const float *qi = q ? q[i] : nullptr, *ri = r ? r[i] : nullptr;
    if ((qi != nullptr) != (ri != nullptr) || (qi != nullptr && yf == nullptr)) return fail(DMM_ERR_INVALID, "q, r and yfwd come together");
    if (d->transposed || d->mode != 0 || d->stride != 1 || d->R * d->S <= 1 || !d->bn_relu || !d->use_mfma)
      return fail(DMM_ERR_INVALID, "the transposed form serves unit-stride multi-tap convolutions behind BN+ReLU");
    const int rc = thin_wgrad_setup(d, g, x[i], dy[i], scale[i], shift[i], yf, qi, ri, dw[i], scratch[i], st, v[i].a, v[i].dd, v[i].dp, v[i].rows);
    if (rc) return rc;
    Resolved res;
    if (!wg3_resolve(v[i].a, d->dtype, res)) return fail(DMM_ERR_INVALID, "not a launch wg3.hip takes (16-bit storage, 128 -> 32 channels, 3x3)");
  }
  void* part = nullptr;
  HIPCHK(hipMallocAsync(&part, (size_t)W3_MAX_SLOTS * W3_SLOT_FLOATS * sizeof(float), st));
  for (One& o : v) { o.a.part = (float*)part; o.a.part_slots = W3_MAX_SLOTS; }
  hipError_t e = hipSuccess;
  int nl = 0;
  if (grouped) {
    Wg3Group G;
    for (int i = 0; i < n && e == hipSuccess; ++i) {
      if (wg3_group_add(G, v[i].a, descs[i].dtype)) continue;
      if (G.n > 0) { e = wg3_group_launch(G, st); ++nl; }
      if (e == hipSuccess && !wg3_group_add(G, v[i].a, descs[i].dtype)) e = hipErrorNotSupported;
    }
    if (e == hipSuccess && G.n > 0) { e = wg3_group_launch(G, st); ++nl; }
    if (e == hipSuccess) note_impl(IMPL_WG3);
  } else {
    for (int i = 0; i < n && e == hipSuccess; ++i, ++nl) e = launch_wgrad(v[i].a, descs[i].dtype, true, st, IMPL_WG3);
  }
  hipFreeAsync(part, st);
  HIPCHK(e);
  for (int i = 0; i < n; ++i) {
    const dmm_conv_desc* d = &descs[i];
    HIPCHK(hipMemsetAsync(dw[i], 0, (size_t)d->Cin * d->Cout * d->R * d->S * sizeof(float), st));
    HIPCHK(launch_unpack(v[i].dd, v[i].dp, 1, v[i].rows, d->dtype, 1.0f, st));
  }
  if (launches) *launches = nl;
  return DMM_OK;
}

int dmm_bw1_reduce_grouped(int n, const float* const* part, float* const* dpack, const int* nct, const int* nsplit, const int* wc,
                           int grouped, int* launches, void* stream) {
  if (n < 1 || !part || !dpack || !nct || !nsplit || !wc) return fail(DMM_ERR_INVALID, "null argument");
  hipStream_t st = (hipStream_t)stream;
  Bw1RedGroup G;
  int nl = 0;
  for (int i = 0; i < n; ++i) {
    if (!part[i] || !dpack[i] || nct[i] < 1 || nsplit[i] < 1 || wc[i] < 1 || wc[i] > nct[i] * 128 || wc[i] <= (nct[i] - 1) * 128)
      return fail(DMM_ERR_INVALID, "a member needs slots, a packed gradient, nct, nsplit >= 1 and (nct - 1) * 128 < wc <= nct * 128");
    Bw1RedMember m;
    m.part = part[i]; m.dpack = dpack[i]; m.nct = nct[i]; m.nsplit = nsplit[i];
    m.nfloats = ((wc[i] + 31) / 32) * 128 * 32;
    if (!grouped) { HIPCHK(launch_bw1_reduce_member(m, st)); ++nl; continue; }
    if (G.n >= B1_RED_GROUP_MAX) { HIPCHK(bw1_reduce_group_launch(G, st)); ++nl; }
    G.m[G.n++] = m;
  }
  if (G.n > 0) { HIPCHK(bw1_reduce_group_launch(G, st)); ++nl; }
  if (launches) *launches = nl;
  return DMM_OK;
}

}
```

### dmmfods_amd/csrc/plan.cpp

```cpp
#include "plan.h"

#include <algorithm>
#include <cmath>
#include <cstdio>
#include <cstdlib>
#include <cstring>
#include <map>
#include <stdexcept>

namespace dmm {

static unsigned tw1(int mt) { return 0xffffff00u | (unsigned)mt; }

std::vector<Tap> taps_conv(int R, int S, int pad) {
  std::vector<Tap> t;
  for (int ky = 0; ky < R; ++ky)
    for (int kx = 0; kx < S; ++kx) t.push_back({ky - pad, kx - pad, tw1(ky * S + kx)});
  return t;
}
std::vector<Tap> taps_conv_dgrad(int R, int S, int pad) {
  std::vector<Tap> t;
  for (int ky = 0; ky < R; ++ky)
    for (int kx = 0; kx < S; ++kx) t.push_back({pad - ky, pad - kx, tw1(ky * S + kx)});
  return t;
// ... 164 lines not shown
  for (int j = 0; j < g.nb; ++j) {
    const std::string p = "decoder.Transposed_Convolution_Sequence_" + std::to_string(j + 1);
    tb.bn(p + ".norm0", g.nin[j]);
    tb.add(p + ".conv_reduce.weight", DMM_T_CONV, {g.nf[j], g.nin[j], 1, 1});
    tb.bn(p + ".norm1", g.nf[j]);
    tb.add("decoder.Transposed_Convolution_" + std::to_string(j + 1) + ".weight", DMM_T_CONVT, {g.nf[j], g.nf[j], 3, 3});
  }
  const int nfl = g.nf[g.nb - 1], hin = nfl + g.s1 + g.s2;
  tb.bn("dec_out_to_heat_maps.norm0", hin);
  tb.add("dec_out_to_heat_maps.refine0.weight", DMM_T_CONV, {nfl / 2, hin, 3, 3});
  tb.bn("dec_out_to_heat_maps.norm1", nfl / 2);
  tb.add("dec_out_to_heat_maps.refine1.weight", DMM_T_CONV, {g.nc, nfl / 2, 5, 5});
  if (g.fusion == 2) {
    encoder_table(tb, "stream_2_features", g, g.s2, g.cbb - 1);
    const int c = g.cin[g.cbb - 1];
    tb.bn("concat_module.norm", 2 * c);
    tb.add("concat_module.conv.weight", DMM_T_CONV, {c, 2 * c, 1, 1});
  }
  np = tb.np;
  nbuf = tb.nb;
}

namespace {

struct Bump {
  size_t off = 0;
  size_t take(size_t bytes, size_t align = 256) {
    off = (off + align - 1) / align * align;
    const size_t o = off;
    off += bytes;
    return o;
  }
};

struct Buf {
  int B, H, W, ld;
  int cw = 0;
  uint8_t* x = nullptr;
  uint8_t* g = nullptr;
  double* ssum = nullptr;
  double* ssq = nullptr;
  float* q = nullptr;
  float* r = nullptr;
  float* ql = nullptr;
  float* rl = nullptr;
  double* qd = nullptr;
  double* rd = nullptr;
  bool ginit = false;
  bool matz = false;
  bool materialized = false;
  int front = 0;
  int mat_front = 0;
};

struct BnRange { int buf, ch0, c0, n; double count, count_unb; bool want_qr; };
struct Bn {
  int C;
  float *gamma, *beta, *rm, *rv, *dgamma, *dbeta;
  float *scale, *shift, *mean, *invstd;
  double *red1, *red2;
  int cp = 0;
  std::vector<BnRange> ranges;
};

enum DgradKind { DG_NONE = 0, DG_FLIP, DG_POOL2, DG_CONVT, DG_UP2 };

struct SegRec {
  int buf, ch0, C , Cw , koff, mode, istride;
  int bn, bn_c0;
  int dgrad;
};
struct PhaseRec { int py, px; std::vector<Tap> taps; int pack; std::vector<Tap> taps1;  };
struct ConvRec {
  std::string wname;
  bool transposed;
  int N, Kin, R, S, pad;
  int B, Ho, Wo;
  int nseg;
  SegRec seg[2];
  int obuf, och0, ostride;
  int epi;
  bool stats;
  std::vector<PhaseRec> phases;
  int dpack[2];
  bool wgrad_transposed;
  bool shared_master;
  double flops_ref;
};
struct PoolRec { int y0buf, bn, obuf, och0; uint8_t* argmax; int C; };
struct Rec { int type; int idx; };
struct BucketRec {
  int64_t off = 0, n = 0;
  int convs_left = 0, bns_left = 0;
  int first_desc = 0, ndesc = 0, rows = 0;
  int tile0 = 0, nt1 = 0, nt9 = 0;
  int last_main = -1, last_side = -1;
};

enum LaunchRole { ROLE_STORE, ROLE_BNBWD, ROLE_LOGITS, ROLE_WGRAD , ROLE_WGRAD_T  };
const char* launch_class(int impl, LaunchRole role) {
  static const struct { LaunchRole role; int impl; const char* cls; } table[] = {
      {ROLE_STORE, IMPL_CONV3, "conv3.store"}, {ROLE_STORE, IMPL_CVP, "cvp.store"},     {ROLE_STORE, IMPL_CF, "cf.store"},
      {ROLE_STORE, IMPL_HALO, "halo.store"},   {ROLE_STORE, IMPL_PIG, "pig.store"},     {ROLE_STORE, IMPL_HF, "hf.store"},
      {ROLE_STORE, IMPL_AUTO, "igemm.store"},  {ROLE_BNBWD, IMPL_CONV3, "conv3.bnbwd"}, {ROLE_BNBWD, IMPL_CVP, "cvp.bnbwd"},
      {ROLE_BNBWD, IMPL_HALO, "halo.bnbwd"},   {ROLE_BNBWD, IMPL_BW1, "bw1"},           {ROLE_BNBWD, IMPL_AUTO, "igemm.bnbwd"},
      {ROLE_LOGITS, IMPL_THIN, "thin.logits"}, {ROLE_LOGITS, IMPL_HALO, "halo.logits"}, {ROLE_LOGITS, IMPL_AUTO, "igemm.logits"},
      {ROLE_WGRAD, IMPL_WGP, "wgp"},           {ROLE_WGRAD, IMPL_WG5, "wg5"},           {ROLE_WGRAD, IMPL_AUTO, "wgrad"},
      {ROLE_WGRAD_T, IMPL_WG3, "wg3"},         {ROLE_WGRAD_T, IMPL_WG5, "wg5"},         {ROLE_WGRAD_T, IMPL_AUTO, "wgradT"},
  };
  for (auto& row : table)
    if (row.role == role && (row.impl == impl || row.impl == IMPL_AUTO)) return row.cls;
  return "?";
}

struct Builder {
  dmm_plan& P;
  const dmm_model_desc& d;
  Geo g;
  const int dtype, esz, SLOT, BK;
  const bool sizing;
  uint8_t *zbase, *zbbase, *wbase;
  float *Pp, *Pg, *Pb;
  Bump Z, ZB, W;
  float* wg3_part = nullptr;
  bool wg3_part_taken = false;
  std::map<std::string, const TensorInfo*> tmap;
  std::vector<Buf> bufs;
  std::vector<Bn> bns;
  std::vector<ConvRec> convs;
  std::vector<PoolRec> pools;
  std::vector<Rec> recs;
  int in1 = -1, in2 = -1, inH = -1, dl = -1;
  size_t s2_recs = 0, concat_rec = 0;
  double flops = 0;
  PackDesc* pack_dev = nullptr;
  int* prefix_dev = nullptr;
  PackTile* ptiles_dev = nullptr;
  int total_rows = 0;
  int pack_split = 0, pack_rows0 = 0;
  size_t pack_cut_rec = 0;
  int pt_early1 = 0, pt_early9 = 0, pt_late1 = 0, pt_late9 = 0;
  static constexpr double PACK_EARLY_ELEMS = 3.0e6;
  std::vector<BucketRec> brecs;
  PackDesc* unpack_dev = nullptr;
  int* unprefix_dev = nullptr;
  PackTile* utiles_dev = nullptr;
  std::vector<Op>* ops = nullptr;
  bool training = true;
  bool leaf_scope = false;
  bool s2_chain_started = false;
  const bool pack_tiles_on = !P.sw.no_pack_tiles;
  const bool s2_interleave = !P.sw.no_s2_interleave;
  const unsigned deny = P.deny;
  const bool s2_overlap = !lab_flag("DMM_NO_S2_OVERLAP");
  const bool front_matz = !lab_flag("DMM_NO_FRONT_MATZ");
  const int matz_mask = lab_int("DMM_MATZ_MASK", 7);
  const bool pad_pitch = lab_flag("DMM_PITCH_PAD");
  const bool frozen = P.encoder_frozen;
  std::vector<std::pair<int64_t, int64_t>> frozen_ranges;

  static bool is_encoder_name(const std::string& n) {
    return n.rfind("features.", 0) == 0 || n.rfind("stream_2_features.", 0) == 0 || n.rfind("concat_module.", 0) == 0;
  }
  bool frozen_off(int64_t off) const {
    for (auto& r : frozen_ranges)
      if (off >= r.first && off < r.second) return true;
    return false;
  }
  bool is_encoder_rec(const Rec& r) const { return r.type != 0  || is_encoder_name(convs[r.idx].wname); }

  Builder(dmm_plan& p, bool sizing_, uint8_t* ws)
      : P(p), d(p.desc), g(p.desc), dtype(p.desc.dtype), esz((int)dtype_size(p.desc.dtype)), SLOT(16 / esz), BK(4 * (16 / esz)),
        sizing(sizing_) {
    auto fake = [](int k) { return (uint8_t*)(uintptr_t)((0x100ull + (uintptr_t)k) << 40); };
    zbase = sizing ? fake(0) : ws;
    zbbase = sizing ? fake(1) : ws + p.zero_bytes;
    wbase = sizing ? fake(2) : ws + p.zero_bytes + p.zero_bwd_bytes;
    Pp = sizing ? (float*)fake(3) : p.params;
    Pg = sizing ? (float*)fake(4) : p.grads;
    Pb = sizing ? (float*)fake(5) : p.buffers;
    for (auto& t : P.tensors) tmap[t.name] = &t;
    if (frozen)
      for (auto& t : P.tensors) {
        if (t.kind > DMM_T_BN_BIAS || !is_encoder_name(t.name)) continue;
        int64_t n = 1;
        for (int k = 0; k < t.ndim; ++k) n *= t.shape[k];
        if (!frozen_ranges.empty() && frozen_ranges.back().second == t.off) frozen_ranges.back().second += n;
        else frozen_ranges.push_back({t.off, t.off + n});
      }
  }

  template <typename U> U* zptr(size_t n) { return (U*)((uintptr_t)zbase + Z.take(n * sizeof(U))); }
  template <typename U> U* zbptr(size_t n) { return (U*)((uintptr_t)zbbase + ZB.take(n * sizeof(U))); }
  template <typename U> U* wptr(size_t n) { return (U*)((uintptr_t)wbase + W.take(n * sizeof(U))); }
  int rup(int v, int m) const { return (v + m - 1) / m * m; }

  const TensorInfo& T(const std::string& n) {
    auto it = tmap.find(n);
    if (it == tmap.end()) throw std::runtime_error("unknown tensor " + n);
    return *it->second;
  }

  int new_buf(int B, int H, int W_, int cw, bool grad, bool stats, bool matz = false) {
    Buf b;
    b.matz = matz && !lab_flag("DMM_NO_MATZ");
    int ld = cw;
    if (pad_pitch && cw >= 64 && (cw * esz) % 256 == 0) ld = cw + 64 / esz;
    b.B = B; b.H = H; b.W = W_; b.ld = ld; b.cw = cw;
    const size_t n = (size_t)B * H * W_ * ld;
    b.x = wptr<uint8_t>(n * esz);
    if (grad) b.g = wptr<uint8_t>(n * esz);
    if (stats) { b.ssum = zptr<double>((size_t)ld * STAT_REPS); b.ssq = zptr<double>((size_t)ld * STAT_REPS); }
    if (grad) {
      b.q = zbptr<float>(ld + 8); b.r = zbptr<float>(ld + 8); b.ql = zbptr<float>(ld + 8); b.rl = zbptr<float>(ld + 8);
      b.qd = zbptr<double>(ld + 8); b.rd = zbptr<double>(ld + 8);
    }
    bufs.push_back(b);
    return (int)bufs.size() - 1;
  }

  int new_bn(const std::string& prefix, int C) {
    Bn b;
    b.C = C;
    const TensorInfo &w = T(prefix + ".weight"), &bi = T(prefix + ".bias"), &rm = T(prefix + ".running_mean"),
                     &rv = T(prefix + ".running_var");
    b.gamma = Pp + w.off; b.beta = Pp + bi.off;
    b.dgamma = Pg + w.off; b.dbeta = Pg + bi.off;
    b.rm = Pb + rm.off; b.rv = Pb + rv.off;
    const int cp = rup(C, 8) + 8;
    b.scale = wptr<float>(cp); b.shift = wptr<float>(cp); b.mean = wptr<float>(cp); b.invstd = wptr<float>(cp);
    b.red1 = zbptr<double>((size_t)cp * STAT_REPS); b.red2 = zbptr<double>((size_t)cp * STAT_REPS);
    b.cp = cp;
    bns.push_back(b);
    return (int)bns.size() - 1;
  }
  void bn_range(int bn, int buf, int ch0, int c0, int n, double unb_mult = 1.0, bool want_qr = true) {
    const Buf& b = bufs[buf];
    const double cnt = (double)b.B * b.H * b.W;
    bns[bn].ranges.push_back({buf, ch0, c0, n, cnt, cnt * unb_mult, want_qr});
  }

  int add_pack(const ConvRec& c, const std::vector<Tap>& taps, bool dgrad_seg, int seg_index, const std::vector<Tap>* taps1 = nullptr) {
    PackDesc pd;
    memset(&pd, 0, sizeof(pd));
    const TensorInfo& w = T(c.wname);
    pd.w = Pp + w.off;
    const long long RS = (long long)c.R * c.S;
    long long base_off = 0;
    if (!dgrad_seg) {
      pd.N = c.N;
      pd.nseg = c.nseg;
      if (!c.transposed) { pd.sn = c.Kin * RS; pd.sk = RS; }
      else { pd.sn = RS; pd.sk = (long long)c.N * RS; }
      for (int s = 0; s < c.nseg; ++s)
        fill_pack_seg(pd.seg[s], (s == 1 && taps1 && !taps1->empty()) ? *taps1 : taps, c.seg[s].Cw, c.seg[s].C, c.seg[s].koff, BK);
      pd.gw = Pg + w.off;
      pd.shared_master = c.shared_master ? 1 : 0;
    } else {
      const SegRec& sr = c.seg[seg_index];
      pd.N = sr.Cw;
      pd.nseg = 1;
      if (!c.transposed) { pd.sn = RS; pd.sk = c.Kin * RS; base_off = sr.koff * RS; }
      else { pd.sn = (long long)c.N * RS; pd.sk = RS; }
      const int kc = rup(c.N, 8);
      fill_pack_seg(pd.seg[0], taps, c.N, kc, 0, BK);
    }
    pd.st = 1;
    pd.rs = (int)RS;
    pd.w += base_off;
    {
      const int cs = dgrad_seg ? c.seg[seg_index].C : 0;
      pd.Npad = dgrad_seg ? rup(cs, cs >= 384 || cs % 128 == 0 ? 128 : (cs >= 64 ? 64 : 32)) : rup(c.N, 32);
    }
    int chunks = 0;
    for (int s = 0; s < pd.nseg; ++s) chunks += pd.seg[s].nchunks;
    const size_t elems = (size_t)chunks * pd.Npad * BK;
    pd.dst = wptr<uint8_t>(elems * esz);
    if (!dgrad_seg) pd.dpack = zbptr<float>(elems);
    P.packs.push_back(pd);
    return (int)P.packs.size() - 1;
  }

  Op& push(int kind) {
    ops->emplace_back();
    ops->back().kind = kind;
    ops->back().leaf = leaf_scope ? 1 : 0;
    return ops->back();
  }
  struct LeafScope {
    bool& flag;
    const bool outer;
    LeafScope(Builder& b, bool on) : flag(b.leaf_scope), outer(b.leaf_scope) { flag = on; }
    ~LeafScope() { flag = outer; }
  };
  Op& push(int kind, bool leaf) {
    LeafScope scope(*this, leaf);
    return push(kind);
  }
  bool is_raw_input(int buf) const { return buf == in1 || buf == in2 || buf == inH; }
  void tag(Op& o, const std::string& cls, const std::string& layer, double flops, double bytes) {
    snprintf(o.label, sizeof(o.label), "%s/%s", cls.c_str(), layer.c_str());
    o.flops = flops;
    o.bytes = bytes;
  }
  static std::string ncls(int impl, LaunchRole role, int npad) {
    return std::string(launch_class(impl, role)) + ".n" + std::to_string(npad % 128 == 0 ? 128 : (npad % 64 == 0 ? 64 : 32));
// ... 308 lines not shown
            for (int t = 0; t < 4; ++t) m.w.ph_xtaps[ph][t] = po.w.seg[0].taps[t < po.w.seg[0].ntaps ? t : 0];
            m.w.ph_ntaps[ph] = (signed char)po.w.seg[0].ntaps;
            m.w.ph_ytap[ph] = po.w.dy.taps[0];
            m.w.ph_dpack[ph] = po.w.dpack;
          },
          [&](Op& m) {
            bool all4 = true;
            for (int ph = 0; ph < 4; ++ph) all4 = all4 && m.w.ph_ntaps[ph] == 4;
            if (all4) m.w.ph_ntaps[0] = m.w.ph_ntaps[1] = m.w.ph_ntaps[2] = m.w.ph_ntaps[3] = 0;
            return wgrad_pick(m.w, dtype, d.use_mfma != 0, deny) == IMPL_WGP;
          });
  }

  bool raw_segment_once(const ConvRec& c) const {
    return c.nseg == 2 && c.phases.size() == 4 && c.shared_master && c.seg[1].C == 8 && c.seg[1].istride == 2 && c.ostride == 2 &&
           !lab_flag("DMM_NO_RAW_ONCE");
  }
  void emit_wgrad_raw(ConvRec& c, ConvBwd& st) {
    const Buf& ob = bufs[c.obuf];
    const SegRec& sr = c.seg[1];
    float* raw_sbuf = nullptr;
    if (dtype != DT_F32 && c.N == 64 && !P.sw.no_raw_stats) raw_sbuf = zbptr<float>(W5_SBUF_FLOATS);
    Op& o = push(OP_WGRAD);
    WgradArgs& a = o.w;
    a.nseg = 1;
    fill_fwd_seg(a.seg[0], sr, taps_conv(3, 3, 1));
    a.seg[0].istride = 1;
    a.B = c.B; a.Ho = ob.H; a.Wo = ob.W; a.M = c.B * ob.H * ob.W;
    fill_grad_seg(a.dy, c.obuf, c.och0, rup(c.N, 8), taps_conv(1, 1, 0), 1);
    one_tap_seg(a.dy, 0, 0);
    const PackDesc& pd = P.packs[c.phases[0].pack];
    a.N = c.N; a.Npad = pd.Npad;
    a.dpack = (float*)pd.dpack + (size_t)pd.seg[0].nchunks * pd.Npad * BK;
    o.impl = wgrad_pick(a, dtype, d.use_mfma != 0, deny);
    if (raw_sbuf != nullptr && o.impl == IMPL_WG5 && sr.bn >= 0) {
      WgradArgs f = a;
      f.sbuf = raw_sbuf;
      f.t_mean = bns[sr.bn].mean + sr.bn_c0;
      f.t_invstd = bns[sr.bn].invstd + sr.bn_c0;
      if (wgrad_pick(f, dtype, d.use_mfma != 0, deny) == IMPL_WG5) { a = f; st.raw_stats = true; }
    }
    const Buf& rb = bufs[sr.buf];
    tag(o, ncls(o.impl, ROLE_WGRAD, pd.Npad), short_name(c.wname) + ".raw", conv_flops(c, 1) * ((double)sr.Cw / c.Kin),
        (double)rb.B * rb.H * rb.W * 8 * esz + grad_reads(c) * out_bytes(c));
    if (!st.raw_stats) return;
    const WgradArgs wa = o.w;
    const int leaf_of = o.leaf;
    Op& fo = push(OP_RAWFIN);
    fo.leaf = leaf_of ? leaf_of : 1;
    RawFinArgs& r = fo.rf;
    r.sbuf = wa.sbuf; r.dpack = wa.dpack; r.Npad = wa.Npad;
    r.w = Pp + T(c.wname).off; r.Kin = c.Kin; r.koff = sr.koff; r.nreal = sr.Cw;
    for (int t = 0; t < 9; ++t) r.tapw[t] = (int)(pd.seg[1].tapw[t] & 0xff);
    const Bn& bn = bns[sr.bn];
    r.gamma = bn.gamma + sr.bn_c0; r.beta = bn.beta + sr.bn_c0;
    r.red1 = bn.red1 + sr.bn_c0; r.red2 = bn.red2 + sr.bn_c0;
    tag(fo, "wg5.rawfin", short_name(c.wname) + ".raw", 0, W5_SBUF_FLOATS * 4.0);
  }

  void emit_dgrad_seg(ConvRec& c, int s, ConvBwd& st) {
    const SegRec& sr = c.seg[s];
    const Buf& sb = bufs[sr.buf];
    const bool pool2 = sr.dgrad == DG_POOL2, up = sr.dgrad == DG_CONVT || sr.dgrad == DG_UP2;
    const int rH = pool2 ? sb.H / 2 : sb.H, rW = pool2 ? sb.W / 2 : sb.W;
    const bool raw = is_raw_input(sr.buf);
    Op& o = push(OP_IGEMM, raw);
    o.epi = EPI_BNBWD;
    ConvArgs& a = o.c;
    a.nseg = 1;
    fill_grad_seg(a.seg[0], c.obuf, c.och0, rup(c.N, 8), dgrad_taps(c, sr.dgrad), up ? 2 : 1);
    a.B = sb.B; a.Ho = rH; a.Wo = rW; a.M = sb.B * rH * rW;
    const PackDesc& pd = P.packs[c.dpack[s]];
    a.wpack = pd.dst;
    a.N = sr.C; a.Npad = pd.Npad;
    a.out = raw ? nullptr : gat(sr.buf, sr.ch0);
    a.ldo = sb.ld; a.Hout = sb.H; a.Wout = sb.W; a.ostride = pool2 ? 2 : 1; a.py = 0; a.px = 0;
    a.bx = xat(sr.buf, sr.ch0);
    a.ldbx = sb.ld;
    const Bn& bn = bns[sr.bn];
    a.bscale = bn.scale + sr.bn_c0; a.bshift = bn.shift + sr.bn_c0;
    a.bmean = bn.mean + sr.bn_c0; a.binvstd = bn.invstd + sr.bn_c0;
    a.red1 = bn.red1 + sr.bn_c0; a.red2 = bn.red2 + sr.bn_c0;
    a.stat_stride = bn.cp;
    a.accumulate = (sb.ginit && !raw) ? 1 : 0;
    a.pool2 = pool2 ? 1 : 0;
    const double srcb = (double)sb.B * sb.H * sb.W * sr.C * esz;
    const double segf = conv_flops(c, 1) * ((double)sr.Cw / c.Kin) * (sr.dgrad == DG_UP2 ? 16.0 / 36.0 : 1.0);
    o.impl = igemm_pick(a, dtype, EPI_BNBWD, d.use_mfma != 0, deny);
    if (st.wg3_held && o.impl == IMPL_CONV3) {
      a.eff_out = st.eff_compact;
      Seg& q = st.wg3_op.w.seg[0];
      q.src = st.eff_compact; q.ld = 32;
      q.src2 = nullptr; q.ld2 = 0; q.q = q.r = q.ql = q.rl = nullptr;
    }
    tag(o, ncls(o.impl, ROLE_BNBWD, pd.Npad), short_name(c.wname), segf,
        grad_reads(c) * out_bytes(c) + srcb * (sb.ginit ? 3.0 : 2.0) + w_bytes(c));
  }

  void split_two_pass(ConvRec& c, int s, ConvBwd& st) {
    const SegRec& sr = c.seg[s];
    const Buf& sb = bufs[sr.buf];
    Op& o = ops->back();
    if (!(o.impl == IMPL_CONV3 && !is_raw_input(sr.buf) && sb.matz && sb.q && !sb.ginit && !sb.materialized && is_head5x5(c) && !P.sw.no_two_pass)) return;
    const double srcb = (double)sb.B * sb.H * sb.W * sr.C * esz;
    Op first_pass = o;
    first_pass.c.out = nullptr;
    Op second_pass = o;
    second_pass.c.red1 = nullptr; second_pass.c.red2 = nullptr;
    second_pass.c.eq = sb.q + sr.ch0; second_pass.c.er = sb.r + sr.ch0;
    if (igemm_pick(first_pass.c, dtype, EPI_BNBWD, d.use_mfma != 0, deny) != IMPL_CONV3 ||
        igemm_pick(second_pass.c, dtype, EPI_BNBWD, d.use_mfma != 0, deny) != IMPL_CONV3)
      return;
    st.have_second = true;
    st.second_buf = sr.buf;
    st.second_pass = second_pass;
    st.second_pass.bytes = out_bytes(c) + srcb * 2.0 + w_bytes(c);
    o.c.out = nullptr;
    o.bytes = out_bytes(c) + srcb + w_bytes(c);
    if (st.r1_idx < 0) return;
    const Bn& bn = bns[sr.bn];
    WgradArgs f = (*ops)[st.r1_idx].w;
    f.sbuf = st.r1_sbuf;
    f.t_mean = bn.mean + sr.bn_c0; f.t_invstd = bn.invstd + sr.bn_c0;
    if (wgrad_pick(f, dtype, d.use_mfma != 0, deny) != IMPL_WG5) return;
    Op& wo = (*ops)[st.r1_idx];
    wo.w = f;
    wo.chain = 1;
    const PackDesc& wpd = P.packs[c.dpack[0]];
    Fin64Args r = {};
    r.sbuf = st.r1_sbuf; r.dpack = f.dpack; r.Npad = f.Npad;
    r.w = Pp + T(c.wname).off; r.Kin = c.Kin; r.nreal = c.N; r.dtype = dtype;
    for (int t = 0; t < 25; ++t) r.tapw[t] = (unsigned char)(wpd.seg[0].tapw[t] & 0xff);
    r.scale = bn.scale + sr.bn_c0; r.shift = bn.shift + sr.bn_c0;
    r.mean = bn.mean + sr.bn_c0; r.invstd = bn.invstd + sr.bn_c0;
    r.red1 = bn.red1 + sr.bn_c0; r.red2 = bn.red2 + sr.bn_c0;
    o.kind = OP_FIN64; o.epi = 0; o.impl = IMPL_AUTO; o.chain = 1;
    o.f64 = r;
    tag(o, "wg5.fin64", short_name(c.wname), 0, W5_SBUF64_FLOATS * 4.0);
  }

  void take_back_1x1_wgrad(const ConvRec& c, ConvBwd& st) {
    if (!(d.use_mfma && is_1x1_pair(c) && !ops->empty() && ops->back().kind == OP_WGRAD && !leaf_scope)) return;
    st.w1_op = ops->back();
    ops->pop_back();
    st.w1_held = true;
  }
  void fold_bw1(const ConvRec& c, ConvBwd& st) {
    const bool raw = is_raw_input(c.seg[0].buf);
    const Op dgrad_op = ops->back();
    const Op& saved_w = st.w1_op;
    float* part = nullptr;
    int part_slots = 0;
    if (!raw && dtype != DT_F32 && c.N == 128) {
      const Bw1Geom q = bw1_geometry(dgrad_op.c);
      part_slots = q.nsplit * q.nct;
      part = wptr<float>((size_t)part_slots * B1_SLOT_FLOATS);
    }
    if (raw || !bw1_eligible(saved_w.w, dgrad_op.c, dtype, deny)) {
      ops->pop_back();
      ops->push_back(saved_w);
      st.dgrad_op = dgrad_op;
      st.dgrad_behind = true;
      return;
    }
    Op& f = ops->back();
    f.kind = OP_BW1;
    f.b1.dpack = saved_w.w.dpack;
    f.b1.dNpad = saved_w.w.Npad;
    f.b1.wC = saved_w.w.seg[0].C;
    f.b1.part = part;
    f.b1.part_slots = part_slots;
    f.b1.nct = f.b1.ntiles = f.b1.tiles_per_wg = f.b1.xcd_group = f.b1.nsplit = 0;
    tag(f, ncls(IMPL_BW1, ROLE_BNBWD, f.c.Npad), short_name(c.wname), dgrad_op.flops + saved_w.flops, dgrad_op.bytes + w_bytes(c) * 4.0 / esz);
    if (part == nullptr) return;
    const Bw1Args b1 = f.b1;
    Op& rop = push(OP_BW1RED);
    rop.leaf = 1;
    rop.b1 = b1;
    tag(rop, "bw1.reduce", short_name(c.wname), 0, ((double)part_slots + b1.nct) * B1_SLOT_FLOATS * 4.0);
  }

  void emit_conv_bwd(ConvRec& c) {
    ConvBwd st;
    if (c.wgrad_transposed) {
      emit_wgrad_thin(c, st);
    } else {
      const bool raw_once = raw_segment_once(c);
      emit_wgrad_phases(c, raw_once ? 1 : c.nseg);
      if (raw_once) emit_wgrad_raw(c, st);
      take_back_1x1_wgrad(c, st);
    }
    if (!st.wgrad_side_open()) conv_grad_done(c);
    for (int s = 0; s < c.nseg; ++s) {
      const SegRec& sr = c.seg[s];
      if (sr.dgrad == DG_NONE) continue;
      if (st.raw_stats && s == 1 && is_raw_input(sr.buf)) continue;
      emit_dgrad_seg(c, s, st);
      split_two_pass(c, s, st);
      if (st.w1_held) fold_bw1(c, st);
      if (!is_raw_input(sr.buf)) bufs[sr.buf].ginit = true;
    }
    if (st.wg3_held) ops->push_back(st.wg3_op);
    if (st.wgrad_side_open()) conv_grad_done(c);
    if (st.dgrad_behind) ops->push_back(st.dgrad_op);
    if (st.have_second) bufs[st.second_buf].materialized = true;
    int done = -1;
    for (int s = 0; s < c.nseg; ++s) {
      const int bn = c.seg[s].bn;
      if (bn < 0 || bn == done || c.seg[s].dgrad == DG_NONE) continue;
      emit_bn_bwd_finalize(bn);
      done = bn;
    }
    if (st.have_second) ops->push_back(st.second_pass);
  }

  void emit_pool_fwd(PoolRec& p) {
    emit_bn_finalize(p.bn);
    Op& o = push(OP_POOL);
    MaxpoolArgs& a = o.mp;
    const Buf &yb = bufs[p.y0buf], &ob = bufs[p.obuf];
    a.y0 = yb.x; a.ld0 = yb.ld; a.H0 = yb.H; a.W0 = yb.W; a.B = yb.B; a.C = p.C;
    a.scale = bns[p.bn].scale; a.shift = bns[p.bn].shift;
    a.out = (void*)xat(p.obuf, p.och0); a.ldo = ob.ld; a.Hp = ob.H; a.Wp = ob.W;
    a.argmax = p.argmax;
    a.stat_sum = ob.ssum + p.och0; a.stat_sq = ob.ssq + p.och0; a.stat_stride = ob.ld;
    tag(o, "maxpool.fwd", "pool0", 0, ((double)yb.B * yb.H * yb.W + (double)ob.B * ob.H * ob.W) * p.C * esz + (double)ob.B * ob.H * ob.W * p.C);
  }
  void emit_pool_bwd(PoolRec& p) {
    LeafScope leaf(*this, true);
    Op& o = push(OP_POOLBWD);
    MaxpoolBwdArgs& a = o.mpb;
    Buf &yb = bufs[p.y0buf];
    const Buf &ob = bufs[p.obuf];
    a.y0 = yb.x; a.ld0 = yb.ld; a.H0 = yb.H; a.W0 = yb.W; a.B = yb.B; a.C = p.C;
    a.scale = bns[p.bn].scale; a.shift = bns[p.bn].shift;
    a.gpool = gat(p.obuf, p.och0); a.xpool = xat(p.obuf, p.och0);
    a.q = ob.q + p.och0; a.r = ob.r + p.och0; a.ql = ob.ql + p.och0; a.rl = ob.rl + p.och0;
    a.ldg = ob.ld; a.Hp = ob.H; a.Wp = ob.W;
    a.argmax = p.argmax;
    a.gy0 = yb.g;
    a.mean = bns[p.bn].mean; a.invstd = bns[p.bn].invstd;
    a.red1 = bns[p.bn].red1; a.red2 = bns[p.bn].red2; a.stat_stride = bns[p.bn].cp;
    tag(o, "maxpool.bwd", "pool0", 0, (2.0 * yb.B * yb.H * yb.W + 2.0 * ob.B * ob.H * ob.W) * p.C * esz + (double)ob.B * ob.H * ob.W * p.C);
    yb.ginit = true;
    emit_bn_bwd_finalize(p.bn);
  }

  ConvRec& new_conv(const std::string& wname, bool transposed, int N, int Kin, int R, int S, int pad) {
    ConvRec c;
    c.wname = wname; c.transposed = transposed; c.N = N; c.Kin = Kin; c.R = R; c.S = S; c.pad = pad;
    c.nseg = 1; c.ostride = 1; c.epi = EPI_STORE; c.stats = true;
    c.dpack[0] = c.dpack[1] = -1;
    c.wgrad_transposed = false;
    c.shared_master = false;
    c.flops_ref = 0;
    memset(c.seg, 0, sizeof(c.seg));
    c.seg[0].bn = c.seg[1].bn = -1;
    convs.push_back(c);
    recs.push_back({0, (int)convs.size() - 1});
    return convs.back();
  }
  void finish_conv(ConvRec& c) {
    for (auto& ph : c.phases) ph.pack = add_pack(c, ph.taps, false, 0, &ph.taps1);
    for (int s = 0; s < c.nseg; ++s) {
      if (c.seg[s].dgrad != DG_NONE) c.dpack[s] = add_pack(c, dgrad_taps(c, c.seg[s].dgrad), true, s);
    }
    if (c.nseg == 1 && !c.transposed && c.seg[0].mode == G_PLAIN && c.seg[0].istride == 1 && c.seg[0].dgrad == DG_FLIP &&
        c.R * c.S > 1 && rup(c.N, 8) < c.seg[0].C && c.phases.size() == 1) {
      c.wgrad_transposed = true;
      PackDesc& dp = P.packs[c.dpack[0]];
      int chunks = 0;
      for (int s2 = 0; s2 < dp.nseg; ++s2) chunks += dp.seg[s2].nchunks;
      dp.dpack = zbptr<float>((size_t)chunks * dp.Npad * BK);
      dp.gw = Pg + (dp.w - Pp);
      P.packs[c.phases[0].pack].gw = nullptr;
    }
    flops += conv_flops(c, 1);
  }
  void plain_conv(const std::string& wname, int N, int Kin, int R, int pad, int buf, int ch0, int mode, int istride, int bn, int dgrad,
                  int Ho, int Wo, int obuf, int och0) {
    ConvRec& c = new_conv(wname, false, N, Kin, R, R, pad);
    set_seg(c, 0, buf, ch0, Kin, 0, mode, istride, bn, 0, dgrad);
    c.B = bufs[buf].B; c.Ho = Ho; c.Wo = Wo; c.obuf = obuf; c.och0 = och0;
    c.phases.push_back({0, 0, taps_conv(R, R, pad), -1});
    finish_conv(c);
  }
  void set_seg(ConvRec& c, int s, int buf, int ch0, int Cw, int koff, int mode, int istride, int bn, int bn_c0, int dgrad) {
    SegRec& sr = c.seg[s];
    sr.buf = buf; sr.ch0 = ch0; sr.Cw = Cw; sr.C = rup(Cw, 8); sr.koff = koff; sr.mode = mode; sr.istride = istride;
    sr.bn = bn; sr.bn_c0 = bn_c0; sr.dgrad = dgrad;
  }

  void stem(const std::string& p, int inbuf, int in_ch, int obuf, int och0) {
    const Buf ib = bufs[inbuf];
    const int y0 = new_buf(ib.B, ib.H / 2, ib.W / 2, g.nif, true, true);
    plain_conv(p + ".conv0.weight", g.nif, in_ch, 7, 3, inbuf, 0, G_PLAIN, 2, -1, DG_NONE, ib.H / 2, ib.W / 2, y0, 0);
    PoolRec pr;
    pr.y0buf = y0;
    pr.bn = new_bn(p + ".norm0", g.nif);
    bn_range(pr.bn, y0, 0, 0, g.nif);
    pr.obuf = obuf; pr.och0 = och0; pr.C = g.nif;
    pr.argmax = wptr<uint8_t>((size_t)ib.B * (ib.H / 4) * (ib.W / 4) * g.nif);
    pools.push_back(pr);
    recs.push_back({1, (int)pools.size() - 1});
  }

  void dense_block(const std::string& p, int xb, int base, int b) {
    const Buf X = bufs[xb];
    const int bw = g.bs * g.k;
    for (int l = 0; l < g.L[b]; ++l) {
      const std::string q = p + ".denselayer" + std::to_string(l + 1);
      const int K = g.cin[b] + l * g.k;
      static const int matz_k = lab_int("DMM_MATZ_DENSE_K", 1 << 30);
      const int y1 = new_buf(X.B, X.H, X.W, rup(bw, 8), true, true, K >= matz_k);
      const int n1 = new_bn(q + ".norm1", K);
      bn_range(n1, xb, base, 0, K);
      plain_conv(q + ".conv1.weight", bw, K, 1, 0, xb, base, G_PLAIN, 1, n1, DG_FLIP, X.H, X.W, y1, 0);
      const int n2 = new_bn(q + ".norm2", bw);
      bn_range(n2, y1, 0, 0, bw);
      plain_conv(q + ".conv2.weight", g.k, bw, 3, 1, y1, 0, G_PLAIN, 1, n2, DG_FLIP, X.H, X.W, xb, base + K);
    }
  }

  void transition(const std::string& p, int xb, int base, int C, int obuf, int och0) {
// ... 491 lines not shown
```

### dmmfods_amd/csrc/plan.h

```cpp
#pragma once
#include <cstring>
#include <stdexcept>
#include <string>
#include <vector>

#include "../../include/dmmfods_hip.h"
#include "common.h"
#include "pointwise.h"

namespace dmm {

struct plan_sizing_error : std::runtime_error { using std::runtime_error::runtime_error; };

struct TensorInfo {
  std::string name;
  int kind, ndim;
  int64_t shape[4];
  int64_t off;
};

struct Tap {
  int dy, dx;
  unsigned tapw;
};

std::vector<Tap> taps_conv(int R, int S, int pad);
std::vector<Tap> taps_conv_dgrad(int R, int S, int pad);
std::vector<Tap> taps_convT_phase(int py, int px);
std::vector<Tap> taps_convT_dgrad();
std::vector<Tap> taps_up2_merged_dgrad();
std::vector<Tap> taps_up2_phase(int e, int f);
std::vector<Tap> taps_conv_phase_s2(int e, int f);
void fill_seg_taps(Seg& s, const std::vector<Tap>& taps, int BK);
void fill_pack_seg(PackSeg& p, const std::vector<Tap>& taps, int Creal, int Cpad, int koff, int BK);

enum OpKind { OP_MEMSET = 0, OP_CONVERT, OP_IGEMM, OP_WGRAD, OP_BNFIN, OP_BNBWD, OP_POOL, OP_POOLBWD, OP_BCE, OP_PACK, OP_UNPACK,
              OP_COPY, OP_APPLYCORR, OP_BW1, OP_JOIN, OP_BW1RED, OP_RAWFIN, OP_FIN64 };

struct MemsetArgs { void* p; size_t bytes; };
struct CopyArgs { void* dst; const void* src; size_t bytes; };
struct PackArgs {
  const PackDesc* descs; const int* prefix; int ndesc, total_rows; float grad_scale;
  const PackDesc* tdescs; const PackTile* tiles; int nt1, nt9;
};

struct Op {
  int kind;
  int epi;
  int leaf;
  int chain;
  int signal;
  int impl;
  double flops;
  double bytes;
  char label[56];
  union {
    MemsetArgs ms;
    CopyArgs cp;
    ConvertArgs cv;
    ConvArgs c;
    WgradArgs w;
    BnFinalizeArgs bf;
    BnBwdFinalizeArgs bb;
    MaxpoolArgs mp;
    MaxpoolBwdArgs mpb;
    BceArgs bce;
    PackArgs pk;
    ApplyCorrArgs ac;
    Bw1Args b1;
    RawFinArgs rf;
    Fin64Args f64;
  };
  Op() { memset(static_cast<void*>(this), 0, sizeof(*this)); signal = -1; impl = IMPL_AUTO; }
};

}

struct GradBucket {
  int64_t off = 0, n = 0;
  int ev_main = -1, ev_side = -1;
  int ready = -1;
};

struct PlanSwitches {
  bool no_pack_tiles = false, no_hf = false, no_c3_merge = false, no_cvp_merge = false, no_wgp_merge = false, no_two_pass = false,
       no_eff_compact = false, no_s2_interleave = false, no_raw_stats = false, no_r1_stats = false;
  int pack_cut = 0;
  static PlanSwitches from_environment();
};

struct dmm_plan {
  dmm_model_desc desc;
  PlanSwitches sw;
  unsigned deny = 0;
  std::vector<dmm::TensorInfo> tensors;
  int64_t nparams = 0, nbuf = 0;
  size_t zero_bytes = 0, zero_bwd_bytes = 0, main_bytes = 0;
  double fwd_flops = 0;
  bool bound = false;
  void* ws = nullptr;
  float *params = nullptr, *grads = nullptr, *buffers = nullptr;
  std::vector<dmm::Op> fwd_train, fwd_eval, bwd;
  std::vector<int> convert_ops_train, convert_ops_eval;
  int logits_op_train = -1, logits_op_eval = -1;
  int bce_op = -1, bce_only_valid = 0;
  dmm::Op bce_only;
  int loss_kind = 0;
  float loss_alpha[8] = {1, 1, 1, 1, 1, 1, 1, 1}, loss_gamma[8] = {2, 2, 2, 2, 2, 2, 2, 2};
  bool grad_accumulate = false;
  bool encoder_frozen = false;
  const float* dyn_scale = nullptr;
  double* metrics = nullptr;
  size_t metrics_bytes = 0;
  std::vector<dmm::PackDesc> packs;
  std::vector<int> pack_prefix;
  std::vector<dmm::PackDesc> unpacks;
  std::vector<int> unpack_prefix;
  std::vector<dmm::PackTile> pack_tiles, unpack_tiles;
  size_t bucket_bytes = 0;
  std::vector<GradBucket> buckets;
  std::vector<void*> bucket_events;
  int prof_max_passes = 0;
  int prof_pass[2] = {0, 0};
  std::vector<std::vector<void*>> prof_events[2];
  std::string prof_filter;
  int device = -1;
  bool used_side = false, used_capture = false;
  std::vector<void*> join_events;
  std::vector<void*> fork_events;
  struct GraphEntry { const void* key[4]; void* exec; unsigned long long stamp; };
  struct GraphCache {
    std::vector<GraphEntry> entries;
    const void* seen[4][4] = {};
    int nseen = 0;
    int captures = 0;
    unsigned long long epoch = 0;
  };
  GraphCache graphs[2];
  bool graph_failed = false;
  bool dp_used = false;
  unsigned long long graph_clock = 0;
  long long graph_replays[2] = {0, 0};
  long long batch_counts[4] = {0, 0, 0, 0};
};
```

### dmmfods_amd/csrc/pointwise.h

```cpp
#pragma once
#include "../../include/dmmfods_hip.h"
#include "common.h"

namespace dmm {

struct ConvertArgs {
  const float* src1;
  const float* src2;
  int C1, C2;
  void* dst;
  int B, H, W;
  double* stat_sum;
  double* stat_sq;
  float scale;
  const float* dyn_scale;
};

struct BnFinalizeArgs {
  const double* sum;
  const double* sq;
  int stat_stride;
  double count;
  double count_unbiased;
  const float* gamma;
// ... 20 lines not shown
  float* dbeta;
  double* qd;
  double* rd;
  float* q;
  float* r;
  float* ql;
  float* rl;
  double count;
  float grad_scale;
  int C;
  int accumulate;
};

struct MaxpoolArgs {
  const void* y0;
  int ld0, H0, W0, B, C;
  const float* scale;
  const float* shift;
  void* out;
  int ldo, Hp, Wp;
  unsigned char* argmax;
  double* stat_sum;
  double* stat_sq;
  int stat_stride;
};

struct MaxpoolBwdArgs {
  const void* y0;
  int ld0, H0, W0, B, C;
  const float* scale;
  const float* shift;
  const void* gpool;
  const void* xpool;
  const float* q;
  const float* r;
  const float* ql;
  const float* rl;
  const float* mean;
  const float* invstd;
  int ldg, Hp, Wp;
  const unsigned char* argmax;
  void* gy0;
  double* red1;
  double* red2;
  int stat_stride;
};

struct BceArgs {
  const float* logits;
  const float* target;
  void* dlogits;
  double* out;
  int B, NC, H, W;
  float thr, loss_scale;
  int kind, from_prob;
  float alpha[8], gamma[8];
  float* loss_out;
  float* dx_out;
  int metrics;
  const float* dyn_scale;
};

struct ApplyCorrArgs {
  void* g;
  const void* y;
  const float* q;
  const float* r;
  const float* ql;
  const float* rl;
  size_t npix;
  int C, ldg, ldy;
};

struct AdamArgs {
  float* p;
  const float* g;
  float* m;
  float* v;
  size_t n;
  float beta1, beta2, eps, weight_decay, step_size, bc2_sqrt, grad_scale;
};

constexpr int GUARD_PARTIALS = 512;
struct GradSumsqArgs {
  const float* g;
  size_t n;
  double* partials;
  int accumulate;
};
constexpr int ADAM_MAX_CLASSES = DMM_ADAM_MAX_CLASSES;
constexpr int ADAM_SEG_CHUNK = 1024;
constexpr int ADAM_SEG_MAX_GRID = 2048;
struct AdamSegDev {
  long long begin, end;
  int cls, pad;
};
struct AdamSegClass {
  float lr, beta1, beta2, eps;
  float weight_decay;
  float decay;
  float step_size, bc2_sqrt;
  long long t0;
  int decoupled;
  int active;
};
struct AdamSegArgs {
  float* p;
  const float* g;
  float* m;
  float* v;
  size_t n;
  const AdamSegDev* segs;
  const int* first;
  int nsegs, nchunks, nclasses;
  int vec_ok;
  float grad_scale;
  const dmm_guard_state* state;
  AdamSegClass cls[ADAM_MAX_CLASSES];
};
struct GuardFinalizeArgs {
  const double* partials;
  dmm_guard_state* state;
  float lr, beta1, beta2;
  float max_norm;
  float growth_factor, backoff_factor;
  int growth_interval;
};

struct PackSeg {
  int Creal, Cpad, ntaps, nchunks, koff;
  unsigned tapw[MAX_TAPS];
};

struct PackDesc {
  const float* w;
  void* dst;
  float* gw;
  const float* dpack;
  int N, Npad, nseg;
  int shared_master;
  long long sn, sk, st;
  PackSeg seg[2];
  int rs;
  int tiled;
};
struct PackTile { int desc, nsib, n0, cg; };

struct Bw1Args {
  ConvArgs c;
  float* dpack;
  int dNpad, wC;
  float* part;
  int part_slots;
  int nct, ntiles, tiles_per_wg, xcd_group, nsplit;
};
struct Bw1Geom { int nct, ntiles, tiles_per_wg, nsplit, xcd_group, nwg; };
Bw1Geom bw1_geometry(const ConvArgs& a);
constexpr int B1_SLOT_FLOATS = 4 * 128 * 32;
bool bw1_eligible(const WgradArgs& w, const ConvArgs& d, int dtype, unsigned deny);
hipError_t launch_bw1(const Bw1Args& g, int dtype, hipStream_t st);
hipError_t launch_bw1_reduce(const Bw1Args& g, hipStream_t st);
constexpr int B1_RED_GROUP_MAX = 32;
struct Bw1RedMember { const float* part; float* dpack; int nct, nsplit, nfloats; };
struct Bw1RedGroup { int n = 0; Bw1RedMember m[B1_RED_GROUP_MAX]; };
bool bw1_reduce_group_add(Bw1RedGroup& G, const Bw1Args& g);
hipError_t bw1_reduce_group_launch(Bw1RedGroup& G, hipStream_t st);
hipError_t launch_bw1_reduce_member(const Bw1RedMember& m, hipStream_t st);
constexpr int W3_GROUP_MAX = 32;
struct Wg3Group {
  int n = 0, dtype = 0, pq = 0, part_slots = 0;
  long long tiles = 0;
  alignas(16) unsigned char block[4096];
};
bool wg3_group_add(Wg3Group& G, const WgradArgs& a, int dtype);
hipError_t wg3_group_launch(Wg3Group& G, hipStream_t st);
hipError_t launch_igemm(const ConvArgs& a, int dtype, int epi, bool mfma, hipStream_t st, int impl = IMPL_AUTO, unsigned deny = 0);
hipError_t launch_wgrad(WgradArgs a, int dtype, bool mfma, hipStream_t st, int impl = IMPL_AUTO, unsigned deny = 0);
int igemm_pick(const ConvArgs& a, int dtype, int epi, bool mfma, unsigned deny);
int wgrad_pick(const WgradArgs& a, int dtype, bool mfma, unsigned deny);
hipError_t launch_wg5_rawfin(const RawFinArgs& a, hipStream_t st);
hipError_t launch_wg5_fin64(const Fin64Args& a, hipStream_t st);
hipError_t launch_convert_input(const ConvertArgs& a, int dtype, hipStream_t st);
hipError_t launch_bn_finalize(const BnFinalizeArgs& a, hipStream_t st);
hipError_t launch_bn_bwd_finalize(const BnBwdFinalizeArgs& a, hipStream_t st);
hipError_t launch_maxpool_fwd(const MaxpoolArgs& a, int dtype, hipStream_t st);
hipError_t launch_maxpool_bwd(const MaxpoolBwdArgs& a, int dtype, hipStream_t st);
hipError_t launch_bce_metrics(const BceArgs& a, int dtype, hipStream_t st);
hipError_t launch_adam(const AdamArgs& a, hipStream_t st);
hipError_t launch_grad_sumsq(const GradSumsqArgs& a, hipStream_t st);
hipError_t launch_guard_finalize(const GuardFinalizeArgs& a, hipStream_t st);
hipError_t launch_adam_guarded(const AdamArgs& a, const dmm_guard_state* state, hipStream_t st);
hipError_t launch_adam_guarded_from(const AdamArgs& a, const dmm_guard_state* state, float lr, int64_t t0, hipStream_t st);
hipError_t launch_adam_segmented(const AdamSegArgs& a, hipStream_t st);
hipError_t launch_guard_init(dmm_guard_state* dev, float scale, int64_t applied, int32_t tracker, hipStream_t st);
hipError_t launch_apply_corr(const ApplyCorrArgs& a, int dtype, hipStream_t st);
hipError_t launch_pack(const PackDesc* descs_dev, const int* prefix_dev, int ndesc, int total_rows, int dtype, hipStream_t st,
                       const PackDesc* tile_descs = nullptr, const PackTile* tiles_dev = nullptr, int nt1 = 0, int nt9 = 0);
hipError_t launch_unpack(const PackDesc* descs_dev, const int* prefix_dev, int ndesc, int total_rows, int dtype, float grad_scale,
                         hipStream_t st, const PackDesc* tile_descs = nullptr, const PackTile* tiles_dev = nullptr, int nt1 = 0, int nt9 = 0,
                         bool accumulate = false);

#if defined(__HIPCC__)
template <bool COH>
__device__ __forceinline__ double stat_load(const double* p) {
  if constexpr (COH) return __hip_atomic_load(p, __ATOMIC_RELAXED, __HIP_MEMORY_SCOPE_AGENT);
  else return *p;
}

template <bool COH>
__device__ __forceinline__ void bn_finalize_channel(const BnFinalizeArgs& a, int c) {
  float mean, var;
  if (a.training) {
    double su = stat_load<COH>(a.sum + c), sq = stat_load<COH>(a.sq + c);
    if (a.stat_stride)
      for (int k = 1; k < STAT_REPS; ++k) { su += stat_load<COH>(a.sum + c + (size_t)k * a.stat_stride); sq += stat_load<COH>(a.sq + c + (size_t)k * a.stat_stride); }
    const double m = su / a.count;
    double v = sq / a.count - m * m;
    if (v < 0) v = 0;
    mean = (float)m;
    var = (float)v;
    const double unb = a.count_unbiased > 1 ? v * (a.count_unbiased / (a.count_unbiased - 1.0)) : v;
    a.running_mean[c] = (1.f - a.momentum) * a.running_mean[c] + a.momentum * mean;
    a.running_var[c] = (1.f - a.momentum) * a.running_var[c] + a.momentum * (float)unb;
  } else {
    mean = a.running_mean[c];
    var = a.running_var[c];
  }
  const float invstd = 1.0f / sqrtf(var + a.eps);
  const float s = a.gamma[c] * invstd;
  a.scale[c] = s;
  a.shift[c] = a.beta[c] - mean * s;
  a.mean[c] = mean;
  a.invstd[c] = invstd;
}

template <bool COH>
__device__ __forceinline__ void bn_bwd_finalize_channel(const BnBwdFinalizeArgs& a, int c) {
  double S1 = stat_load<COH>(a.red1 + c), S2 = stat_load<COH>(a.red2 + c);
  if (a.stat_stride)
    for (int k = 1; k < STAT_REPS; ++k) { S1 += stat_load<COH>(a.red1 + c + (size_t)k * a.stat_stride); S2 += stat_load<COH>(a.red2 + c + (size_t)k * a.stat_stride); }
  const double mu = a.mean[c], is = a.invstd[c];
  const double dotp = S2;
  const float dg = (float)(dotp * a.grad_scale), db = (float)(S1 * a.grad_scale);
  if (a.accumulate) {
    a.dgamma[c] += dg;
    a.dbeta[c] += db;
  } else {
    a.dgamma[c] = dg;
    a.dbeta[c] = db;
  }
  if (a.qd != nullptr) {
    const double s = a.scale[c];
    const double c1 = S1 / a.count, c2 = dotp / a.count;
    const double q = a.qd[c] + (-s * c1 + s * c2 * mu * is);
    const double r = a.rd[c] + (-s * c2 * is);
    a.qd[c] = q;
    a.rd[c] = r;
    const float qh = (float)q, rh = (float)r;
    a.q[c] = qh; a.ql[c] = (float)(q - (double)qh);
    a.r[c] = rh; a.rl[c] = (float)(r - (double)rh);
  }
}

#endif

}
```

### include/dmmfods_hip.h

```cpp
#ifndef DMMFODS_HIP_H
#define DMMFODS_HIP_H
#include <stddef.h>
#include <stdint.h>

#ifdef __cplusplus
extern "C" {
#endif

typedef enum {
  DMM_OK = 0,
  DMM_ERR_INVALID = -1,
  DMM_ERR_SHAPE = -2,
  DMM_ERR_HIP = -3,
  DMM_ERR_STATE = -4,
  DMM_ERR_NO_DEVICE = -5
} dmm_status;

enum { DMM_F32 = 0, DMM_F16 = 1, DMM_BF16 = 2 };

enum { DMM_T_CONV = 0, DMM_T_CONVT = 1, DMM_T_BN_WEIGHT = 2, DMM_T_BN_BIAS = 3, DMM_T_BN_MEAN = 4, DMM_T_BN_VAR = 5,
       DMM_T_BN_TRACKED = 6 };

typedef struct {
  int32_t growth_rate;
  int32_t num_blocks;
  int32_t block_config[8];
  int32_t num_init_features;
  int32_t bn_size;
  int32_t num_classes;
  int32_t concat_before_block_num;
  int32_t stream_1_in_channels;
  int32_t stream_2_in_channels;
  int32_t batch, height, width;
  int32_t dtype;
  float loss_scale;
  float bn_momentum, bn_eps;
  float iou_threshold;
  int32_t use_mfma;
} dmm_model_desc;

typedef struct dmm_plan dmm_plan;

const char* dmm_last_error(void);
int dmm_version(void);
int dmm_set_option(const char* name, int value);

int dmm_plan_create(const dmm_model_desc* desc, dmm_plan** out);
int dmm_plan_destroy(dmm_plan* plan);

int dmm_plan_num_tensors(const dmm_plan* plan);
int dmm_plan_tensor_info(const dmm_plan* plan, int index, const char** name, int32_t* kind, int32_t* ndim,
                         int64_t shape[4], int64_t* arena_offset);
int64_t dmm_plan_num_params(const dmm_plan* plan);
int64_t dmm_plan_num_buffer_elems(const dmm_plan* plan);
size_t dmm_plan_workspace_bytes(const dmm_plan* plan);
double dmm_plan_forward_flops(const dmm_plan* plan);

int dmm_plan_bind(dmm_plan* plan, void* workspace, size_t workspace_bytes, float* params, float* grads, float* buffers);

int dmm_plan_forward(dmm_plan* plan, const float* stream_1, const float* stream_2, float* logits_out, int training,
                     void* stream);

int dmm_plan_loss_backward(dmm_plan* plan, const float* logits, const float* target, double* metrics_out, void* stream);

enum { DMM_LOSS_BCE = 0, DMM_LOSS_FOCAL = 1 };
int dmm_plan_set_loss(dmm_plan* plan, int kind, const float* alpha, const float* gamma, int nclass);

int dmm_loss_forward(int kind, int from_prob, const float* alpha, const float* gamma, const float* input, const float* target,
                     float* loss_out, float* dinput_out, int batch, int nclass, int height, int width, void* stream);

int dmm_plan_backward(dmm_plan* plan, const float* dlogits, void* stream);

int dmm_plan_set_grad_accumulate(dmm_plan* plan, int accumulate);

int dmm_plan_set_encoder_frozen(dmm_plan* plan, int frozen);

int dmm_plan_num_grad_buckets(const dmm_plan* plan);
int dmm_plan_grad_bucket(const dmm_plan* plan, int index, int64_t* offset, int64_t* count);
int dmm_plan_grad_bucket_wait(dmm_plan* plan, int index, void* stream);

int dmm_plan_profile_begin(dmm_plan* plan, int max_passes);
int dmm_plan_profile_filter(dmm_plan* plan, const char* label_prefix);
int dmm_plan_profile_num_ops(const dmm_plan* plan, int which);
int dmm_plan_profile_op(const dmm_plan* plan, int which, int index, const char** label, double* flops, double* bytes);
int dmm_plan_profile_collect(dmm_plan* plan, int which, double* ms_sum, int n, int* passes);

int dmm_plan_loss_metrics(dmm_plan* plan, const float* logits, const float* target, double* metrics_out, void* stream);

long long dmm_plan_num_graph_replays(const dmm_plan* plan, int which);
int dmm_plan_wgrad_batch_counts(const dmm_plan* plan, long long counts[4]);

int dmm_adam_step(float* params, const float* grads, float* exp_avg, float* exp_avg_sq, int64_t n, float lr, float beta1,
                  float beta2, float eps, float weight_decay, int64_t step, float grad_scale, void* stream);

typedef struct dmm_guard_state {
  float scale;
  float grad_scale;
  double sumsq;
  float grad_norm;
  int32_t found_inf;
  int64_t applied_steps;
  int64_t skipped_steps;
  int32_t growth_tracker;
  float step_size;
  float bc2_sqrt;
  float clip_coef;
  int32_t reserved[2];
} dmm_guard_state;

size_t dmm_grad_guard_scratch_bytes(int64_t n);
int dmm_guard_state_init(dmm_guard_state* dev, float init_scale, int64_t applied_steps, int32_t growth_tracker, void* stream);
int dmm_adam_step_guarded(float* params, const float* grads, float* exp_avg, float* exp_avg_sq, int64_t n, float lr, float beta1,
                          float beta2, float eps, float weight_decay, float max_norm, float growth_factor, float backoff_factor,
                          int32_t growth_interval, dmm_guard_state* state, void* scratch, void* stream);
int dmm_adam_step_guarded_ranges(float* params, const float* grads, float* exp_avg, float* exp_avg_sq, const int64_t* offsets,
                                 const int64_t* counts, const int64_t* t0, int nranges, float lr, float beta1, float beta2, float eps,
                                 float weight_decay, float max_norm, float growth_factor, float backoff_factor, int32_t growth_interval,
                                 dmm_guard_state* state, void* scratch, void* stream);
int dmm_grad_sumsq(const float* grads, int64_t offset, int64_t count, int accumulate, void* scratch, void* stream);
#define DMM_ADAM_MAX_CLASSES 16
typedef struct dmm_adam_segment {
  int64_t begin, count;
  int32_t cls;
} dmm_adam_segment;
typedef struct dmm_adam_class {
  float lr, beta1, beta2, eps, weight_decay;
  int32_t decoupled;
  int64_t t0;
} dmm_adam_class;
size_t dmm_adam_table_bytes(int nsegs, int64_t n);
int dmm_adam_table_init(void* table_dev, const dmm_adam_segment* segs, int nsegs, int64_t n, int nclasses, void* stream);
int dmm_adam_step_segmented(float* params, const float* grads, float* exp_avg, float* exp_avg_sq, int64_t n, const void* table_dev,
                            int nsegs, const dmm_adam_class* classes, int nclasses, int64_t step, float grad_scale, void* stream);
int dmm_adam_step_guarded_segmented(float* params, const float* grads, float* exp_avg, float* exp_avg_sq, int64_t n,
                                    const void* table_dev, int nsegs, const dmm_adam_class* classes, int nclasses, float max_norm,
                                    float growth_factor, float backoff_factor, int32_t growth_interval, dmm_guard_state* state,
                                    void* scratch, void* stream);
int dmm_plan_set_dynamic_loss_scale(dmm_plan* plan, const float* scale_dev);

typedef struct {
  int32_t dtype, use_mfma;
  int32_t B, H, W;
  int32_t Cin, Cout;
  int32_t R, S, stride, pad;
  int32_t transposed;
  int32_t mode;
  int32_t bn_relu;
} dmm_conv_desc;

size_t dmm_conv_scratch_bytes(const dmm_conv_desc* d);
int dmm_conv_forward(const dmm_conv_desc* d, const void* x, const float* w, const float* scale, const float* shift, void* y,
                     double* stats, void* scratch, void* stream);
int dmm_conv_wgrad(const dmm_conv_desc* d, const void* x, const void* dy, const float* scale, const float* shift, float* dw,
                   void* scratch, void* stream);
int dmm_conv_dgrad(const dmm_conv_desc* d, const void* x, const void* dy, const float* w, const float* scale, const float* shift,
                   void* gx, double* red, void* scratch, void* stream);


int dmm_conv_wgrad_ex(const dmm_conv_desc* d, const void* x, const void* dy, const float* scale, const float* shift, const void* yfwd,
                      const float* q, const float* r, int transposed_form, float* dw, void* scratch, void* stream);
int dmm_conv_dgrad_ex(const dmm_conv_desc* d, const void* x, const void* dy, const float* w, const float* scale, const float* shift,
                      const void* yfwd, const float* q, const float* r, void* gx, int accumulate, double* red, void* scratch,
                      void* stream);
int dmm_conv5_wgrad_stats(const dmm_conv_desc* d, const void* x, const void* dy, const float* w, const float* scale, const float* shift,
                          float* dw, double* red, void* scratch, void* stream);
int dmm_conv1x1_backward_fused(const dmm_conv_desc* d, const void* x, const void* dy, const float* w, const float* scale,
                               const float* shift, const void* yfwd, const float* q, const float* r, void* gx, int accumulate,
                               float* dw, double* red, void* scratch, void* stream);

int dmm_conv_wgrad_grouped(const dmm_conv_desc* descs, int n, const void* const* x, const void* const* dy, const float* const* scale,
                           const float* const* shift, const void* const* yfwd, const float* const* q, const float* const* r,
                           float* const* dw, void* const* scratch, int grouped, int* launches, void* stream);
int dmm_bw1_reduce_grouped(int n, const float* const* part, float* const* dpack, const int* nct, const int* nsplit, const int* wc,
                           int grouped, int* launches, void* stream);

int dmm_last_impl(void);
const char* dmm_impl_name(int impl);
unsigned dmm_impl_mask(int reset);

#ifdef __cplusplus
}
#endif
#endif
```

Measured before the change: 159.7 img/s.

## Pair adjacent channel tiles in bw1 workgroups to share the gradient tile

Adds a paired bw1 kernel variant: a 512-thread workgroup covers two adjacent 128-channel tiles and loads and stages the shared dy/gradient operand into LDS once, each half loading only half its rows. The goal is to halve redundant global reads of the gradient (and, with PQ, the forward output) when Cin spans several channel tiles, and to rebalance the split across CUs. This costs more LDS per workgroup and fewer, larger workgroups, which could lower occupancy. It is on by default (pair=1) when nct is even and the grid exceeds the CU count, and it adds geometry and block-map query APIs.

```diff
diff --git a/dmmfods_amd/_lib.py b/dmmfods_amd/_lib.py
--- a/dmmfods_amd/_lib.py
+++ b/dmmfods_amd/_lib.py
@@ -142,6 +142,8 @@
     L.dmm_conv_wgrad_grouped.argtypes = [C.POINTER(ConvDesc), C.c_int, vp, vp, vp, vp, vp, vp, vp, vp, vp, C.c_int, C.POINTER(C.c_int), vp]
     L.dmm_bw1_reduce_grouped.argtypes = [C.c_int, vp, vp, C.POINTER(C.c_int), C.POINTER(C.c_int), C.POINTER(C.c_int), C.c_int,
                                          C.POINTER(C.c_int), vp]
+    L.dmm_bw1_geometry.argtypes = [C.c_int, C.c_int, C.c_int, C.POINTER(C.c_int)]
+    L.dmm_bw1_block_map.argtypes = [C.c_int, C.c_int, C.c_int, C.c_int, C.POINTER(C.c_int)]
     _lib = L
     return L
 
@@ -158,6 +160,7 @@
     "dmm_plan_set_grad_accumulate", "dmm_plan_set_encoder_frozen", "dmm_adam_step_guarded_ranges",
     "dmm_adam_table_bytes", "dmm_adam_table_init", "dmm_adam_step_segmented", "dmm_adam_step_guarded_segmented",
     "dmm_plan_wgrad_batch_counts", "dmm_conv_wgrad_grouped", "dmm_bw1_reduce_grouped",
+    "dmm_bw1_geometry", "dmm_bw1_block_map",
 ]
 
 
diff --git a/dmmfods_amd/csrc/bw1.hip b/dmmfods_amd/csrc/bw1.hip
--- a/dmmfods_amd/csrc/bw1.hip
+++ b/dmmfods_amd/csrc/bw1.hip
@@ -34,38 +34,50 @@
 constexpr int B1_W = 4 * B1_CT * 64;
 constexpr int B1_STAGE = B1_TM * B1_CT * 4;
 static_assert(B1_STAGE == 2 * B1_IMG, "staging aliases the operand images exactly");
-constexpr int B1_LDS = 2 * B1_IMG + B1_W + 2 * B1_CT * 8 + 6 * B1_CT * 4;
+constexpr int B1_RED = 2 * B1_CT * 8;
+constexpr int B1_KC = 6 * B1_CT * 4;
+constexpr int B1_LDS = 2 * B1_IMG + B1_W + B1_RED + B1_KC;
+constexpr int B1P_THREADS = 2 * NTHREADS;
+constexpr int B1P_GI = 3 * B1_IMG;
+constexpr int B1P_W = 4 * B1_IMG;
+constexpr int B1P_RED = B1P_W + 2 * B1_W;
+constexpr int B1P_KC = B1P_RED + 2 * B1_RED;
+constexpr int B1P_LDS = B1P_KC + 2 * B1_KC;
+static_assert(B1P_LDS <= 160 * 1024, "the paired workgroup fits the compute unit's LDS");
 
 __device__ __forceinline__ int b1_swz(int row, int slot) { return ((((slot >> 2) ^ (row & 3)) << 2) | ((slot & 3) ^ ((row >> 2) & 3))); }
 
-template <typename T, int PQ, bool ACC_, bool PART>
-__global__ __launch_bounds__(NTHREADS, 2) void bw1_kernel(const Bw1Args g) {
+template <typename T, int PQ, bool ACC_, bool PART, bool PAIR>
+__device__ __forceinline__ void bw1_body(const Bw1Args& g) {
   constexpr bool ACC = ACC_ && !(B1_DBG & 32);
   constexpr bool UNC = std::is_same<T, f16>::value;
   static_assert(sizeof(T) == 2, "16-bit storage");
   typedef typename TT<T>::vec V;
   constexpr int SLOT = 8;
   constexpr int NL = B1_TM * 16 / NTHREADS;
+  constexpr int NLG = PAIR ? NL / 2 : NL;
+  constexpr int GROWS = PAIR ? 32 : 16;
   const ConvArgs& a = g.c;
   const Seg& sg = a.seg[0];
 
   extern __shared__ __attribute__((aligned(16))) unsigned char smem[];
-  unsigned char* Ai = smem;
-  unsigned char* Gi = smem + B1_IMG;
-  unsigned char* Wi = smem + 2 * B1_IMG;
-  double* red = (double*)(smem + 2 * B1_IMG + B1_W);
-  float* kc = (float*)(smem + 2 * B1_IMG + B1_W + 2 * B1_CT * 8);
-
-  const int tid = threadIdx.x, lane = tid & 63, wave = tid >> 6;
+  const int half = PAIR ? __builtin_amdgcn_readfirstlane((int)(threadIdx.x >> 8)) : 0;
+  unsigned char* Ai = smem + (PAIR ? half * B1_STAGE : 0);
+  unsigned char* Gi = smem + (PAIR ? B1P_GI : B1_IMG);
+  unsigned char* Wi = smem + (PAIR ? B1P_W + half * B1_W : 2 * B1_IMG);
+  double* red = (double*)(smem + (PAIR ? B1P_RED + half * B1_RED : 2 * B1_IMG + B1_W));
+  float* kc = (float*)(smem + (PAIR ? B1P_KC + half * B1_KC : 2 * B1_IMG + B1_W + B1_RED));
+
+  const int tid = threadIdx.x & (NTHREADS - 1), lane = tid & 63, wave = tid >> 6;
   const int r = lane & 31, h = lane >> 5;
-  const int xcd = blockIdx.x & 7, q = blockIdx.x >> 3;
-  const int ct = g.xcd_group ? q % g.nct : (int)(blockIdx.x % g.nct);
-  const int split = g.xcd_group ? (q / g.nct) * 8 + xcd : (int)(blockIdx.x / g.nct);
+  const Bw1Block bm = bw1_block_map((int)blockIdx.x, g.nct, g.nsplit, g.xcd_group, PAIR ? 1 : 0);
+  if (bm.nslices == 0) return;
+  const int ct = bm.slice + half, split = bm.split;
   const int c0 = ct * B1_CT;
   const int t_beg = split * g.tiles_per_wg, t_end = min(g.ntiles, t_beg + g.tiles_per_wg);
-  if (t_beg >= t_end) return;
 
   const int cs = tid & 15, p0 = tid >> 4;
+  const int gp0 = (int)(threadIdx.x >> 4);
   const int cx = c0 + cs * SLOT;
   const bool cvalid = cx < a.N;
   if (tid < B1_CT) {
@@ -82,6 +94,7 @@
   const unsigned xcol = (unsigned)(cvalid ? cx : 0) * 2u, gcol = (unsigned)(cs * SLOT) * 2u;
   const unsigned xpitch = (unsigned)a.ldbx * 2u, gpitch = (unsigned)sg.ld * 2u, ypitch = (unsigned)sg.ld2 * 2u, opitch = (unsigned)a.ldo * 2u;
   const int lds0 = p0 * 256 + (b1_swz(p0, cs) << 4);
+  const int ldsg0 = PAIR ? gp0 * 256 + (b1_swz(gp0, cs) << 4) : lds0;
 
   {
     const T* wp = (const T*)a.wpack;
@@ -100,8 +113,19 @@
   if (tid < 2 * B1_CT) red[tid] = 0.0;
   __syncthreads();
 
-  V rx[NL], rg[NL], ry[PQ == 2 ? NL : 1];
-  unsigned okp = 0;
+  V rx[NL], rg[NLG], ry[PQ == 2 ? NLG : 1];
+  unsigned okp = 0, okg = 0;
+  auto issue_g = [&](int tile) {
+    okg = 0;
+#pragma unroll
+    for (int i = 0; i < NLG; ++i) {
+      const int m = tile * B1_TM + gp0 + GROWS * i;
+      if (m < a.M) okg |= 1u << i;
+      const unsigned mm = (B1_DBG & 16) ? 0u : (unsigned)min(m, a.M - 1);
+      rg[i] = *(const V*)(gbase + (size_t)(mm * gpitch + gcol));
+      if constexpr (PQ == 2) ry[i] = *(const V*)(ybase + (size_t)(mm * ypitch + gcol));
+    }
+  };
   auto issue = [&](int tile) {
     okp = 0;
 #pragma unroll
@@ -111,8 +135,27 @@
       const unsigned mm = (B1_DBG & 16) ? 0u : (unsigned)min(m, a.M - 1);
       if (B1_NT & 1) rx[i] = __builtin_nontemporal_load((const V*)(xbase + (size_t)(mm * xpitch + xcol)));
       else rx[i] = *(const V*)(xbase + (size_t)(mm * xpitch + xcol));
-      rg[i] = *(const V*)(gbase + (size_t)(mm * gpitch + gcol));
-      if constexpr (PQ == 2) ry[i] = *(const V*)(ybase + (size_t)(mm * ypitch + gcol));
+      if constexpr (!PAIR) {
+        rg[i] = *(const V*)(gbase + (size_t)(mm * gpitch + gcol));
+        if constexpr (PQ == 2) ry[i] = *(const V*)(ybase + (size_t)(mm * ypitch + gcol));
+      }
+    }
+    if constexpr (PAIR) issue_g(tile); else okg = okp;
+  };
+  auto stage_g = [&](auto full_tag, unsigned okgt) {
+    constexpr bool FULL = decltype(full_tag)::value;
+    V z;
+#pragma unroll
+    for (int e = 0; e < SLOT; ++e) z[e] = (T)0;
+    SlotK<SLOT> kg;
+    kg.k0 = 0.f; kg.k1 = 0.f; kg.k2 = 0.f; kg.k3 = 0.f;
+    if (PQ == 2) { kg.k0 = load_fv<SLOT>(kc + 4 * B1_CT + cs * SLOT); kg.k1 = load_fv<SLOT>(kc + 5 * B1_CT + cs * SLOT); }
+#pragma unroll
+    for (int i = 0; i < NLG; ++i) {
+      const bool v = FULL || ((okgt >> i) & 1) != 0;
+      V gv = rg[i];
+      if constexpr (PQ == 2) gv = eff_grad_slot(rg[i], ry[i], kg);
+      *(V*)(Gi + ldsg0 + (GROWS * 256) * i) = v ? gv : z;
     }
   };
 
@@ -140,7 +183,7 @@
   for (int tile = t_beg; tile < t_end; ++tile) {
     V xraw[NL], gold[ACC ? NL : 1];
     const bool full = (tile + 1) * B1_TM <= a.M;
-    const unsigned okt = okp;
+    const unsigned okt = okp, okgt = okg;
     auto stage = [&](auto full_tag) {
       constexpr bool FULL = decltype(full_tag)::value;
       V z;
@@ -157,18 +200,7 @@
           *(V*)(Ai + lds0 + 4096 * i) = v ? av_ : z;
         }
       }
-      {
-        SlotK<SLOT> kg;
-        kg.k0 = 0.f; kg.k1 = 0.f; kg.k2 = 0.f; kg.k3 = 0.f;
-        if (PQ == 2) { kg.k0 = load_fv<SLOT>(kc + 4 * B1_CT + cs * SLOT); kg.k1 = load_fv<SLOT>(kc + 5 * B1_CT + cs * SLOT); }
-#pragma unroll
-        for (int i = 0; i < NL; ++i) {
-          const bool v = FULL || ((okt >> i) & 1) != 0;
-          V gv = rg[i];
-          if constexpr (PQ == 2) gv = eff_grad_slot(rg[i], ry[i], kg);
-          *(V*)(Gi + lds0 + 4096 * i) = v ? gv : z;
-        }
-      }
+      stage_g(full_tag, okgt);
     };
     if (UNC && full) stage(std::true_type()); else stage(std::false_type());
     __syncthreads();
@@ -239,7 +271,7 @@
         for (int i = 0; i < 16; ++i) sa += accd[t][i];
       if (sa == 1.2345e33f) obase[0] = 1;
     } else {
-    float* Cs = (float*)smem;
+    float* Cs = (float*)Ai;
 #pragma unroll
     for (int t = 0; t < 2; ++t)
 #pragma unroll
@@ -339,7 +371,17 @@
 }
 
 template <typename T, int PQ, bool ACC, bool PART>
-static hipError_t launch_bw1_t(const Bw1Args& g, int nwg, hipStream_t st) {
+__global__ __launch_bounds__(NTHREADS, 2) void bw1_kernel(const Bw1Args g) {
+  bw1_body<T, PQ, ACC, PART, false>(g);
+}
+template <typename T, int PQ, bool ACC, bool PART>
+__global__ __launch_bounds__(B1P_THREADS, 2) void bw1_pair_kernel(const Bw1Args g) {
+  bw1_body<T, PQ, ACC, PART, true>(g);
+}
+
+template <typename T, int PQ, bool ACC, bool PART>
+static hipError_t launch_bw1_t(const Bw1Args& g, int nwg, bool paired, hipStream_t st) {
+  if (paired) return launch_lds<bw1_pair_kernel<T, PQ, ACC, PART>>(B1P_LDS, nwg, B1P_THREADS, B1P_LDS, st, g);
   return launch_lds<bw1_kernel<T, PQ, ACC, PART>>(B1_LDS, nwg, NTHREADS, B1_LDS, st, g);
 }
 
@@ -360,20 +402,29 @@
   return true;
 }
 
-Bw1Geom bw1_geometry(const ConvArgs& a) {
+static void bw1_split(Bw1Geom& q, int units, int nsplit0) {
+  const int nsplit = std::min(std::max(1, nsplit0), std::max(1, q.ntiles / 4));
+  q.tiles_per_wg = (q.ntiles + nsplit - 1) / nsplit;
+  q.nsplit = (q.ntiles + q.tiles_per_wg - 1) / q.tiles_per_wg;
+  q.xcd_group = (units > 1 && q.nsplit >= 32 && q.tiles_per_wg >= 8) ? 1 : 0;
+  q.nwg = q.xcd_group ? ((q.nsplit + 7) / 8) * 8 * units : q.nsplit * units;
+}
+
+Bw1Geom bw1_geometry(int M, int Cin, int pair) {
   Bw1Geom q;
-  q.nct = (a.N + B1_CT - 1) / B1_CT;
-  q.ntiles = (a.M + B1_TM - 1) / B1_TM;
+  q.nct = (Cin + B1_CT - 1) / B1_CT;
+  q.ntiles = (M + B1_TM - 1) / B1_TM;
+  q.paired = 0;
   constexpr int cus = DESIGN_CUS;
   static const int per_cu = lab_int("DMM_BW1_PER_CU", 2);
-  int nsplit = std::max(1, (per_cu * cus + q.nct - 1) / q.nct);
-  nsplit = std::min(nsplit, std::max(1, q.ntiles / 4));
-  q.tiles_per_wg = (q.ntiles + nsplit - 1) / nsplit;
-  q.nsplit = (q.ntiles + q.tiles_per_wg - 1) / q.tiles_per_wg;
-  q.xcd_group = (q.nct > 1 && q.nsplit >= 32 && q.tiles_per_wg >= 8) ? 1 : 0;
-  q.nwg = q.xcd_group ? ((q.nsplit + 7) / 8) * 8 * q.nct : q.nsplit * q.nct;
+  bw1_split(q, q.nct, (per_cu * cus + q.nct - 1) / q.nct);
+  if (pair != 0 && q.nct % 2 == 0 && (pair == 2 || q.nsplit * q.nct > cus)) {
+    q.paired = 1;
+    bw1_split(q, q.nct / 2, cus / (q.nct / 2));
+  }
   return q;
 }
+Bw1Geom bw1_geometry(const ConvArgs& a, int pair) { return bw1_geometry(a.M, a.N, pair); }
 
 static bool g_bw1_part = !lab_flag("DMM_NO_BW1_PART");
 
@@ -385,18 +436,19 @@
   Bw1Args g = g0;
   const ConvArgs& a = g.c;
   if (a.M <= 0) return hipSuccess;
-  const Bw1Geom q = bw1_geometry(a);
+  const Bw1Geom q = bw1_geometry(a, g.pair);
   note_impl(IMPL_BW1);
   g.nct = q.nct; g.ntiles = q.ntiles; g.tiles_per_wg = q.tiles_per_wg; g.xcd_group = q.xcd_group; g.nsplit = q.nsplit;
   const int nwg = q.nwg;
   const int pq = a.seg[0].q ? 2 : 0;
   const bool acc = a.accumulate != 0;
   const bool part = bw1_uses_part(g, q);
+  const bool paired = q.paired != 0;
 #define B1_GO(T) \
-  (part ? (pq ? (acc ? launch_bw1_t<T, 2, true, true>(g, nwg, st) : launch_bw1_t<T, 2, false, true>(g, nwg, st))     \
-              : (acc ? launch_bw1_t<T, 0, true, true>(g, nwg, st) : launch_bw1_t<T, 0, false, true>(g, nwg, st)))    \
-        : (pq ? (acc ? launch_bw1_t<T, 2, true, false>(g, nwg, st) : launch_bw1_t<T, 2, false, false>(g, nwg, st))   \
-              : (acc ? launch_bw1_t<T, 0, true, false>(g, nwg, st) : launch_bw1_t<T, 0, false, false>(g, nwg, st))))
+  (part ? (pq ? (acc ? launch_bw1_t<T, 2, true, true>(g, nwg, paired, st) : launch_bw1_t<T, 2, false, true>(g, nwg, paired, st))     \
+              : (acc ? launch_bw1_t<T, 0, true, true>(g, nwg, paired, st) : launch_bw1_t<T, 0, false, true>(g, nwg, paired, st)))    \
+        : (pq ? (acc ? launch_bw1_t<T, 2, true, false>(g, nwg, paired, st) : launch_bw1_t<T, 2, false, false>(g, nwg, paired, st))   \
+              : (acc ? launch_bw1_t<T, 0, true, false>(g, nwg, paired, st) : launch_bw1_t<T, 0, false, false>(g, nwg, paired, st))))
   if (dtype == DT_F16) return B1_GO(f16);
   return B1_GO(bf16);
 #undef B1_GO
@@ -437,7 +489,7 @@
 static bool bw1_reduce_member(const Bw1Args& g, Bw1RedMember& m) {
   const ConvArgs& a = g.c;
   if (a.M <= 0) return false;
-  const Bw1Geom q = bw1_geometry(a);
+  const Bw1Geom q = bw1_geometry(a, g.pair);
   if (!bw1_uses_part(g, q)) return false;
   m.part = g.part; m.dpack = g.dpack; m.nct = q.nct; m.nsplit = q.nsplit;
   m.nfloats = ((g.wC + 31) / 32) * g.dNpad * 32;
diff --git a/dmmfods_amd/csrc/capi.cpp b/dmmfods_amd/csrc/capi.cpp
--- a/dmmfods_amd/csrc/capi.cpp
+++ b/dmmfods_amd/csrc/capi.cpp
@@ -38,6 +38,7 @@
 static int g_batch_wgrad = 1;
 static int g_bucket_mb = getenv("DMM_GRAD_BUCKET_MB") ? atoi(getenv("DMM_GRAD_BUCKET_MB")) : 25;
 static std::atomic<unsigned> g_family_off{lab_family_off()};
+static std::atomic<int> g_bw1_pair{1};
 static unsigned plan_deny(const dmm_plan* p) { return (p->sw.no_hf ? 1u << IMPL_HF : 0u) | g_family_off; }
 
 namespace {
@@ -120,6 +121,11 @@
   if (std::string(name) == "batch_wgrad") {
     if (value < 0 || value > 2) return fail(DMM_ERR_INVALID, "batch_wgrad must be 0, 1 or 2");
     g_batch_wgrad = value;
+    return DMM_OK;
+  }
+  if (std::string(name) == "bw1_pair") {
+    if (value < 0 || value > 2) return fail(DMM_ERR_INVALID, "bw1_pair must be 0, 1 or 2");
+    g_bw1_pair = value;
     return DMM_OK;
   }
   for (const auto& o : kFamilyOptions)
@@ -149,6 +155,7 @@
   p->sw = PlanSwitches::from_environment();
   p->bucket_bytes = (size_t)g_bucket_mb << 20;
   p->deny = plan_deny(p);
+  p->bw1_pair = g_bw1_pair;
   try {
     plan_build_tables(p);
   } catch (const std::domain_error& e) {
@@ -237,6 +244,7 @@
   plan->buffers = buffers;
   plan->graphs[0].epoch = plan->graphs[1].epoch = 0;
   plan->bound = false;
+  plan->bw1_pair = g_bw1_pair;
   plan->deny = plan_deny(plan);
   try {
     plan_bind(plan, workspace);
@@ -741,6 +749,7 @@
   if (on == plan->encoder_frozen) return DMM_OK;
   plan->encoder_frozen = on;
   plan->deny = plan_deny(plan);
+  plan->bw1_pair = g_bw1_pair;
   try {
     plan_size(plan);
   } catch (const std::exception& e) {
@@ -1406,7 +1415,8 @@
   if (!bw1_eligible(wa, b.c, d->dtype, g_family_off)) return fail(DMM_ERR_INVALID, "not a pair bw1.hip fuses (16-bit storage, 128 output channels, Cin % 32 == 0)");
   b.dpack = wa.dpack; b.dNpad = wa.Npad; b.wC = wa.seg[0].C;
   {
-    const Bw1Geom q = bw1_geometry(b.c);
+    b.pair = g_bw1_pair;
+    const Bw1Geom q = bw1_geometry(b.c, b.pair);
     b.part_slots = q.nsplit * q.nct;
     void* part = nullptr;
     HIPCHK(hipMallocAsync(&part, (size_t)b.part_slots * B1_SLOT_FLOATS * sizeof(float), st));
@@ -1471,6 +1481,26 @@
   return DMM_OK;
 }
 
+int dmm_bw1_geometry(int M, int Cin, int pair, int out[6]) {
+  if (M < 1 || Cin < 1 || pair < 0 || pair > 2 || !out) return fail(DMM_ERR_INVALID, "dmm_bw1_geometry: M, Cin >= 1, pair 0..2 and an output array");
+  const Bw1Geom q = bw1_geometry(M, Cin, pair);
+  out[0] = q.nct; out[1] = q.nsplit; out[2] = q.tiles_per_wg; out[3] = q.xcd_group; out[4] = q.nwg; out[5] = q.paired;
+  return DMM_OK;
+}
+
+int dmm_bw1_block_map(int M, int Cin, int pair, int block, int out[4]) {
+  if (M < 1 || Cin < 1 || pair < 0 || pair > 2 || !out) return fail(DMM_ERR_INVALID, "dmm_bw1_block_map: M, Cin >= 1, pair 0..2 and an output array");
+  const Bw1Geom q = bw1_geometry(M, Cin, pair);
+  if (block < 0 || block >= q.nwg) return fail(DMM_ERR_INVALID, "dmm_bw1_block_map: block out of range");
+  const Bw1Block b = bw1_block_map(block, q.nct, q.nsplit, q.xcd_group, q.paired);
+  out[0] = out[1] = out[2] = out[3] = 0;
+  if (b.nslices == 0) return DMM_OK;
+  out[0] = b.split * q.tiles_per_wg * 64;
+  out[1] = std::min(M, (b.split + 1) * q.tiles_per_wg * 64);
+  out[2] = b.slice; out[3] = b.nslices;
+  return DMM_OK;
+}
+
 int dmm_bw1_reduce_grouped(int n, const float* const* part, float* const* dpack, const int* nct, const int* nsplit, const int* wc,
                            int grouped, int* launches, void* stream) {
   if (n < 1 || !part || !dpack || !nct || !nsplit || !wc) return fail(DMM_ERR_INVALID, "null argument");
diff --git a/dmmfods_amd/csrc/plan.cpp b/dmmfods_amd/csrc/plan.cpp
--- a/dmmfods_amd/csrc/plan.cpp
+++ b/dmmfods_amd/csrc/plan.cpp
@@ -340,6 +340,7 @@
   const bool pack_tiles_on = !P.sw.no_pack_tiles;
   const bool s2_interleave = !P.sw.no_s2_interleave;
   const unsigned deny = P.deny;
+  const int bw1_pair = P.bw1_pair;
   const bool s2_overlap = !lab_flag("DMM_NO_S2_OVERLAP");
   const bool front_matz = !lab_flag("DMM_NO_FRONT_MATZ");
   const int matz_mask = lab_int("DMM_MATZ_MASK", 7);
@@ -954,8 +955,8 @@
     float* part = nullptr;
     int part_slots = 0;
     if (!raw && dtype != DT_F32 && c.N == 128) {
-      const Bw1Geom q = bw1_geometry(dgrad_op.c);
-      part_slots = q.nsplit * q.nct;
+      const Bw1Geom q = bw1_geometry(dgrad_op.c, 0), qp = bw1_geometry(dgrad_op.c, 2);
+      part_slots = std::max(q.nsplit, qp.nsplit) * q.nct;
       part = wptr<float>((size_t)part_slots * B1_SLOT_FLOATS);
     }
     if (raw || !bw1_eligible(saved_w.w, dgrad_op.c, dtype, deny)) {
@@ -972,6 +973,7 @@
     f.b1.wC = saved_w.w.seg[0].C;
     f.b1.part = part;
     f.b1.part_slots = part_slots;
+    f.b1.pair = bw1_pair;
     f.b1.nct = f.b1.ntiles = f.b1.tiles_per_wg = f.b1.xcd_group = f.b1.nsplit = 0;
     tag(f, ncls(IMPL_BW1, ROLE_BNBWD, f.c.Npad), short_name(c.wname), dgrad_op.flops + saved_w.flops, dgrad_op.bytes + w_bytes(c) * 4.0 / esz);
     if (part == nullptr) return;
diff --git a/dmmfods_amd/csrc/plan.h b/dmmfods_amd/csrc/plan.h
--- a/dmmfods_amd/csrc/plan.h
+++ b/dmmfods_amd/csrc/plan.h
@@ -93,6 +93,7 @@
   dmm_model_desc desc;
   PlanSwitches sw;
   unsigned deny = 0;
+  int bw1_pair = 1;
   std::vector<dmm::TensorInfo> tensors;
   int64_t nparams = 0, nbuf = 0;
   size_t zero_bytes = 0, zero_bwd_bytes = 0, main_bytes = 0;
diff --git a/dmmfods_amd/csrc/pointwise.h b/dmmfods_amd/csrc/pointwise.h
--- a/dmmfods_amd/csrc/pointwise.h
+++ b/dmmfods_amd/csrc/pointwise.h
@@ -196,10 +196,23 @@
   int dNpad, wC;
   float* part;
   int part_slots;
+  int pair;
   int nct, ntiles, tiles_per_wg, xcd_group, nsplit;
 };
-struct Bw1Geom { int nct, ntiles, tiles_per_wg, nsplit, xcd_group, nwg; };
-Bw1Geom bw1_geometry(const ConvArgs& a);
+struct Bw1Geom { int nct, ntiles, tiles_per_wg, nsplit, xcd_group, nwg, paired; };
+Bw1Geom bw1_geometry(int M, int Cin, int pair);
+Bw1Geom bw1_geometry(const ConvArgs& a, int pair);
+struct Bw1Block { int split, slice, nslices; };
+__host__ __device__ inline Bw1Block bw1_block_map(int block, int nct, int nsplit, int xcd_group, int paired) {
+  const int units = paired ? nct / 2 : nct;
+  const int xcd = block & 7, q = block >> 3;
+  const int u = xcd_group ? q % units : block % units;
+  Bw1Block b;
+  b.split = xcd_group ? (q / units) * 8 + xcd : block / units;
+  b.slice = paired ? 2 * u : u;
+  b.nslices = b.split >= nsplit ? 0 : (paired ? 2 : 1);
+  return b;
+}
 constexpr int B1_SLOT_FLOATS = 4 * 128 * 32;
 bool bw1_eligible(const WgradArgs& w, const ConvArgs& d, int dtype, unsigned deny);
 hipError_t launch_bw1(const Bw1Args& g, int dtype, hipStream_t st);
diff --git a/include/dmmfods_hip.h b/include/dmmfods_hip.h
--- a/include/dmmfods_hip.h
+++ b/include/dmmfods_hip.h
@@ -173,6 +173,8 @@
                            float* const* dw, void* const* scratch, int grouped, int* launches, void* stream);
 int dmm_bw1_reduce_grouped(int n, const float* const* part, float* const* dpack, const int* nct, const int* nsplit, const int* wc,
                            int grouped, int* launches, void* stream);
+int dmm_bw1_geometry(int M, int Cin, int pair, int out[6]);
+int dmm_bw1_block_map(int M, int Cin, int pair, int block, int out[4]);
 
 int dmm_last_impl(void);
 const char* dmm_impl_name(int impl);
```

Result: no change. 160.7 img/s (median of 6 runs) (+0.6%).
